# joeyee/Onet

Measured on AMD Instinct MI355X. Metric: training images/sec (twin 256x256 pass), higher is better.
Workload: dtype f32

## Files before the change

### onet_amd/_lib.py

```python
from __future__ import annotations

import ctypes
import os
import re

HERE = os.path.dirname(os.path.abspath(__file__))
HEADER = os.path.join(os.path.dirname(HERE), "include", "onet_hip.h")
EVAL_HEADER = os.path.join(os.path.dirname(HERE), "include", "onet_hip_eval.h")
RAGGED_HEADER = os.path.join(os.path.dirname(HERE), "include", "onet_hip_ragged.h")
RAGGED_SPLIT_HEADER = os.path.join(os.path.dirname(HERE), "include", "onet_hip_ragged_split.h")
ANYMAP_HEADER = os.path.join(os.path.dirname(HERE), "include", "onet_hip_anymap.h")
PAIRS_HEADER = os.path.join(os.path.dirname(HERE), "include", "onet_hip_pairs.h")
UPMAP_HEADER = os.path.join(os.path.dirname(HERE), "include", "onet_hip_upmap.h")
SPLIT_PAIRS_HEADER = os.path.join(os.path.dirname(HERE), "include", "onet_hip_split_pairs.h")
OPTIM_HEADER = os.path.join(os.path.dirname(HERE), "include", "onet_hip_optim.h")
LIBPATH = os.environ.get("ONET_HIP_LIB") or os.path.join(HERE, "libonet_hip.so")

_CT = {
    "int": ctypes.c_int,
    "int64_t": ctypes.c_int64,
    "uint64_t": ctypes.c_uint64,
    "float": ctypes.c_float,
    "double": ctypes.c_double,
}


def parse_header(path: str = HEADER):
    src = open(path).read()
    src = re.sub(r"/\*.*?\*/", " ", src, flags=re.S)
    src = re.sub(r"//[^\n]*", " ", src)
    src = re.sub(r"^\s*#.*$", " ", src, flags=re.M)
    protos = {}
    for m in re.finditer(r"((?:const\s+)?\w+\s*\*?)\s*(onet_\w+)\s*\(([^)]*)\)\s*;", src):
        ret, name, args = m.group(1).strip(), m.group(2), m.group(3).strip()
        if ret.endswith("*"):
            restype = ctypes.c_char_p if "char" in ret else ctypes.c_void_p
        else:
            restype = _CT[ret]
        argtypes, argnames = [], []
        if args and args != "void":
            for a in args.split(","):
                a = a.strip()
                mm = re.match(r"(?:const\s+)?(\w+)\s*(\*?)\s*(\w+)$", a)
                if not mm:
                    raise ValueError(f"cannot parse argument {a!r} of {name}")
                base, ptr, an = mm.groups()
                argtypes.append(ctypes.c_void_p if ptr else _CT[base])
                argnames.append(an)
        protos[name] = (restype, argtypes, argnames)
    return protos


class OnetHipError(RuntimeError):
    pass


_lib = None
_protos = None


def load(build_if_missing: bool = True):
    global _lib, _protos
    if _lib is not None:
        return _lib
    if not os.path.exists(LIBPATH):
        if not build_if_missing:
            raise OnetHipError(f"{LIBPATH} not built; run `python -m onet_amd.build`")
        from . import build as _build
        _build.build()
    lib = ctypes.CDLL(LIBPATH)
    _protos = {}
    for header in (HEADER, EVAL_HEADER, RAGGED_HEADER, RAGGED_SPLIT_HEADER, ANYMAP_HEADER, PAIRS_HEADER, UPMAP_HEADER, SPLIT_PAIRS_HEADER, OPTIM_HEADER):
        protos = parse_header(header)
        for name, (restype, argtypes, _) in protos.items():
            try:
                fn = getattr(lib, name)
            except AttributeError as e:
                raise OnetHipError(f"libonet_hip.so does not export {name} declared in {os.path.basename(header)}") from e
            fn.restype = restype
            fn.argtypes = argtypes
        _protos.update(protos)
    _lib = lib
    return lib


def last_error() -> str:
    return load().onet_last_error().decode()


PROFILE_HOOK = None


def call(name: str, *args, nbytes=None):
    lib = load()
    hook = PROFILE_HOOK
    tok = hook.begin() if hook is not None else None
    rc = getattr(lib, name)(*args)
    if tok is not None:
        hook.end(name, nbytes, tok)
    if rc != 0:
        raise OnetHipError(f"{name} failed ({rc}): {lib.onet_last_error().decode()}")
    return rc
```

### onet_amd/build.py

```python
import os
import subprocess
import sys

HERE = os.path.dirname(os.path.abspath(__file__))
CSRC = os.path.join(HERE, "csrc")
LIB = os.path.join(HERE, "libonet_hip.so")
SOURCES = ["abi.cpp", "conv_mfma.hip", "conv_wino4.hip", "conv_wino4w.hip", "conv_split.hip", "convt_gemm.hip", "stem.hip", "bn.hip", "spatial.hip", "head_loss.hip", "optim.hip", "evalside.hip", "clutter.hip"]
ARCH = "gfx950"


def _stale():
    if not os.path.exists(LIB):
        return True
    t = os.path.getmtime(LIB)
    deps = [os.path.join(CSRC, f) for f in os.listdir(CSRC) if f.endswith((".hip", ".cpp", ".hpp"))] + \
        [os.path.join(HERE, "..", "include", h) for h in ("onet_hip.h", "onet_hip_eval.h", "onet_hip_ragged.h", "onet_hip_ragged_split.h", "onet_hip_anymap.h", "onet_hip_pairs.h", "onet_hip_upmap.h", "onet_hip_split_pairs.h", "onet_hip_optim.h")]
    return any(os.path.getmtime(d) > t for d in deps)


def build(force=False, verbose=False, variant=None, flags=()):
    lib = LIB if variant is None else os.path.join(HERE, f"libonet_hip_{variant}.so")
    if variant is None and not force and not _stale():
        return LIB
    hipcc = os.environ.get("HIPCC", "/opt/rocm/bin/hipcc")
    objdir = CSRC if variant is None else os.path.join(CSRC, "_" + variant)
    os.makedirs(objdir, exist_ok=True)
    objs = []
    procs = []
    for src in SOURCES:
        obj = os.path.join(objdir, src.rsplit(".", 1)[0] + ".o")
        cmd = [hipcc, "-x", "hip", f"--offload-arch={ARCH}", "-O3", "-fPIC", "-std=c++17", "-Wall",
               "-Wno-unused-result", "-fno-slp-vectorize", *flags, "-c", os.path.join(CSRC, src), "-o", obj]
        if verbose:
            cmd.insert(-4, "-Rpass-analysis=kernel-resource-usage")
        procs.append((src, subprocess.Popen(cmd, stdout=subprocess.PIPE, stderr=subprocess.STDOUT, text=True)))
        objs.append(obj)
    failed = False
    for src, p in procs:
        out, _ = p.communicate()
        if p.returncode != 0:
            failed = True
            sys.stderr.write(f"[onet_amd.build] {src} failed:\n{out}\n")
        elif verbose or out.strip():
            sys.stderr.write(out)
    if failed:
        raise RuntimeError("hipcc failed building libonet_hip.so")
    subprocess.check_call([hipcc, "-shared", "-fPIC", f"--offload-arch={ARCH}", "-o", lib] + objs)
    return lib


if __name__ == "__main__":
    if "--variant" in sys.argv:
        i = sys.argv.index("--variant")
        print(build(variant=sys.argv[i + 1], flags=[a for a in sys.argv[i + 2:]]))
    else:
        print(build(force="--force" in sys.argv, verbose="-v" in sys.argv))
```

### onet_amd/csrc/conv_split.hip

```cpp
#include <algorithm>
#include <cstdlib>
#include "common.hpp"
#include "../../include/onet_hip_ragged.h"
#include "../../include/onet_hip_ragged_split.h"
#include "../../include/onet_hip_anymap.h"
#include "../../include/onet_hip_pairs.h"
#include "../../include/onet_hip_split_pairs.h"

using namespace onet;

typedef float f32x16 __attribute__((ext_vector_type(16)));
typedef __bf16 bf16x8 __attribute__((ext_vector_type(8)));
typedef __bf16 bf16x2 __attribute__((ext_vector_type(2)));
typedef unsigned int u32x4s __attribute__((ext_vector_type(4)));
typedef float f32x4s __attribute__((ext_vector_type(4)));

namespace {

constexpr unsigned OOB_S = 0x80000000u;

__device__ __forceinline__ __amdgpu_buffer_rsrc_t s_rsrc(const void* base, int64_t bytes) {
    const int n = bytes > 0x7fffffffll ? 0x7fffffff : (int)bytes;
    return __builtin_amdgcn_make_buffer_rsrc(const_cast<void*>(base), 0, n, 0x00020000);
}
// ... 383 lines not shown
            }
            __syncthreads();
            buf ^= 1;
        }

        if constexpr (F16) {
#pragma unroll
            for (int m = 0; m < 2; ++m)
#pragma unroll
                for (int n = 0; n < NT; ++n)
#pragma unroll
                    for (int r = 0; r < 16; ++r) acc[m][n][r] *= acc_scale;
        }
        const auto [co0, tx, ty, b, y0, x0] = sp_tile(tile, a.coTiles, a.tilesX, a.tilesY);
        if constexpr (ST) {
            float* sc = reinterpret_cast<float*>(lds + 2 * BUF);
            constexpr float npw = (float)(NT * 32), inv_npw = 1.f / npw;
#pragma unroll
            for (int m = 0; m < 2; ++m)
#pragma unroll
                for (int r = 0; r < 16; ++r) {
                    const int piv = __builtin_bit_cast(int, acc[m][0][r]);
                    const float p0 = __builtin_bit_cast(float, __builtin_amdgcn_readlane(piv, 0));
                    const float p1 = __builtin_bit_cast(float, __builtin_amdgcn_readlane(piv, 32));
                    const float pv = kh ? p1 : p0;
                    float s1 = 0.f, s2 = 0.f;
#pragma unroll
                    for (int n = 0; n < NT; ++n) {
                        const float d = acc[m][n][r] - pv;
                        s1 += d;
                        s2 = fmaf(d, d, s2);
                    }
                    s1 = sp_half_sum(s1);
                    s2 = sp_half_sum(s2);
                    if (l31 == 31) {
                        const int cl = m * 32 + (r & 3) + 8 * (r >> 2) + 4 * kh;
                        sc[(wn * 64 + cl) * 2] = fmaf(s1, inv_npw, pv);
                        sc[(wn * 64 + cl) * 2 + 1] = fmaxf(fmaf(-s1 * inv_npw, s1, s2), 0.f);
                    }
                }
            __syncthreads();
            if (tid < 64 && co0 + tid < a.Cout) {
                float mw[8], qw[8];
#pragma unroll
                for (int w = 0; w < 8; ++w) {
                    mw[w] = sc[(w * 64 + tid) * 2];
                    qw[w] = sc[(w * 64 + tid) * 2 + 1];
                }
                const float mean = 0.125f * (((mw[0] + mw[1]) + (mw[2] + mw[3])) + ((mw[4] + mw[5]) + (mw[6] + mw[7])));
                float m2 = ((qw[0] + qw[1]) + (qw[2] + qw[3])) + ((qw[4] + qw[5]) + (qw[6] + qw[7]));
#pragma unroll
                for (int w = 0; w < 8; ++w) m2 = fmaf(npw * (mw[w] - mean), mw[w] - mean, m2);
                const int64_t nblk = (int64_t)a.B * a.tilesY * a.tilesX;
                const int64_t blk = ((int64_t)b * a.tilesY + ty) * a.tilesX + tx;
                float* sp = a.stats + ((int64_t)(co0 + tid) * nblk + blk) * 3;
                sp[0] = 8.f * npw;
                sp[1] = mean;
                sp[2] = m2;
            }
            __syncthreads();
        }
        float* zb = a.z + (int64_t)b * a.z_bs;
        const int xo = x0 + l31;
#pragma unroll
        for (int m = 0; m < 2; ++m)
#pragma unroll
            for (int n = 0; n < NT; ++n) {
                const int yo = y0 + wn * NT + n;
                if (yo < a.H && xo < a.W) {
#pragma unroll
                    for (int r = 0; r < 16; ++r) {
                        const int co = co0 + m * 32 + (r & 3) + 8 * (r >> 2) + 4 * kh;
                        if (co < a.Cout) zb[(int64_t)co * HW + (int64_t)yo * a.W + xo] = acc[m][n][r];
                    }
                }
            }
    }
}


typedef int i32x4s __attribute__((ext_vector_type(4)));
__device__ __forceinline__ i32x4s sp_rsrc4(const void* base, int64_t bytes) {
    const uint64_t p = reinterpret_cast<uint64_t>(base);
    i32x4s r;
    r.x = (int)(p & 0xffffffffu);
    r.y = (int)((p >> 32) & 0xffffu);
    r.z = bytes > 0x7fffffffll ? 0x7fffffff : (int)bytes;
    r.w = 0x00020000;
    return r;
}
__device__ __forceinline__ void sp_dma16(i32x4s rsrc, unsigned lds_base, unsigned voff, unsigned soff) {
    unsigned keep;
    asm volatile("s_nop 4\n\ts_mov_b32 %0, m0\n\ts_mov_b32 m0, %3\n\ts_nop 0\n\tbuffer_load_dwordx4 %1, %2, %4 offen lds\n\ts_mov_b32 m0, %0"
                 : "=&s"(keep)
                 : "v"(voff), "s"(rsrc), "s"(lds_base), "s"(soff)
                 : "memory");
}

__global__ void split_pack_act_kernel(const float* __restrict__ x, int64_t x_bs, unsigned* __restrict__ xs, int64_t xs_bs, int B, int C8,
                                      int H, int W, int f16, float scale, const unsigned* __restrict__ slots) {
    if (slots) {
        float inv;
        scale *= amax_scale(amax_read(slots), false, inv);
    }
    const int64_t n = (int64_t)B * C8 * H * W;
    for (int64_t i = blockIdx.x * (int64_t)blockDim.x + threadIdx.x; i < n; i += (int64_t)gridDim.x * blockDim.x) {
        const int xx = (int)(i % W);
        int64_t r = i / W;
        const int y = (int)(r % H);
        r /= H;
        const int c8 = (int)(r % C8), b = (int)(r / C8);
        const float* src = x + (int64_t)b * x_bs + ((int64_t)c8 * 8 * H + y) * W + xx;
        u32x4s hi, mid;
#pragma unroll
        for (int c = 0; c < 4; ++c) {
            const float va = src[(int64_t)(2 * c) * H * W] * scale, vb = src[(int64_t)(2 * c + 1) * H * W] * scale;
            unsigned h, m;
            if (f16 == 1) split2h(va, vb, h, m);
            else split2(va, vb, h, m);
            hi[c] = h;
            mid[c] = m;
        }
        if (f16 == 2) {
            reinterpret_cast<u32x4s*>(xs + (int64_t)b * xs_bs)[((int64_t)c8 * H + y) * W + xx] = hi;
            continue;
        }
        u32x4s* dst = reinterpret_cast<u32x4s*>(xs + (int64_t)b * xs_bs) + (((int64_t)c8 * H + y) * 2) * W + xx;
        dst[0] = hi;
        dst[W] = mid;
    }
}

struct SpPreArgs {
    const void* xs;
    int64_t xs_bs;
    const __bf16* wq;
    float* z;
    int64_t z_bs;
    int B, Cin, Cout, H, W, tilesX, tilesY, coTiles;
    float* stats;
    const unsigned* x_slots;
    int x_always;
    const unsigned* x_slots2;
    int split_ch;
    const float* rd_z = nullptr;
    union { int64_t rd_z_bs = 0; int64_t pl_y_bs; };
    const float* rd_save = nullptr;
    union { int rd_gimg = 0; int n_img; };
    float* rd_rec = nullptr;
    unsigned* rd_amax = nullptr;
    int z16 = 0, rd_z16 = 0;
    void* zP = nullptr;
    int64_t zP_bs = 0;
    int zP_ch0 = 0;
    const unsigned* zP_slots = nullptr;
    const float* act_save = nullptr;
    unsigned* act_amax = nullptr;
    float* act_a = nullptr;
    int64_t act_a_bs = 0;
    union { const float* hd_L = nullptr; void* pl_P; };
    union { int64_t hd_L_bs = 0; int64_t pl_P_bs; };
    union { float* hd_V = nullptr; float* pl_y; };
};

template <bool W16> struct SpPreCfg {
    static constexpr int NW = 8, NT = 16 / NW, TW = 32, CO_T = 64, ROWS = NW * NT;
    static constexpr int IN_ROWS = ROWS + 2, IN_COLS = W16 ? 36 : 34;
    static constexpr int NPIX = IN_ROWS * IN_COLS;
    static constexpr int NPIXP = W16 ? 656 : 640;
    static constexpr int W_PART = 9 * 2 * CO_T, W_SLOTS = 2 * W_PART, NWI = (W_SLOTS + NW * 64 - 1) / (NW * 64);
    static constexpr int IN_PART = 2 * NPIXP;
    static constexpr int BUF_SLOTS = W_SLOTS + 2 * IN_PART;
    static constexpr int LDS_BYTES = 2 * BUF_SLOTS * 16;
    static constexpr int NB = (NT - 1) + 3;
    static constexpr int LAST_TAP = 4;
    static_assert(CO_T == SpCfg::CO_T && ROWS == SpCfg::ROWS && TW == SpCfg::TW, "sp_tile: one tile shape for every kernel of the family");
};
template <int CTRL> __device__ __forceinline__ float dpp_max(float x) {
    return fmaxf(x, __builtin_bit_cast(float, __builtin_amdgcn_update_dpp(0, __builtin_bit_cast(int, x), CTRL, 0xf, 0xf, false)));
}
template <bool ST, int PM, bool W16, bool ACT = false, bool POOL = false, bool RAG = false>
__global__ __launch_bounds__(SpPreCfg<W16>::NW * 64, SpPreCfg<W16>::NW / 4) void conv3x3_split_pre_kernel(SpPreArgs a) {
    constexpr bool F16 = PM == 1;
    static_assert(!RAG || ACT, "conv3x3_split_pre_kernel: the ragged instance is the activation epilogue's (masked exact maximum)");
    static_assert(!ACT || (PM == 1 && !ST && (!W16 || (RAG && !POOL))),
                  "conv3x3_split_pre_kernel: the activation epilogue goes with the fp16 slot store; on image-pair tiles: the masked record, no pooled twin");
    static_assert(!POOL || ACT, "conv3x3_split_pre_kernel: the pooled stores ride on the activation epilogue");
    using C = SpPreCfg<W16>;
    constexpr bool PAIRS = W16 && ACT;
    constexpr int NT = C::NT, IN_COLS = C::IN_COLS, NWI = C::NWI, CO_T = C::CO_T, NPIXP = C::NPIXP, NB = C::NB;
    constexpr int BUF = C::BUF_SLOTS, W_PART = C::W_PART, IN_PART = C::IN_PART;
    constexpr int NWV = C::NW, NTH = NWV * 64;
    constexpr int NII = (2 * IN_PART + NTH - 1) / NTH;
    extern __shared__ __attribute__((aligned(16))) unsigned char smem_s[];
    u32x4s* lds = reinterpret_cast<u32x4s*>(smem_s);

    int t_first, t_end, t_stride;
    sp_tile_range(a.tilesX * a.tilesY * a.B * a.coTiles, t_first, t_end, t_stride);
    if (t_first >= t_end) return;

    const int tid = threadIdx.x, lane = tid & 63, wn = __builtin_amdgcn_readfirstlane(tid >> 6);
    const int l31 = lane & 31, kh = lane >> 5;
    const int HW = a.H * a.W;
    const int nchunks = PM == 2 ? a.Cin >> 5 : a.Cin >> 4;

    const i32x4s wr = sp_rsrc4(a.wq, (int64_t)a.Cin * (PM == 2 ? 1 : 2) * 9 * a.Cout * 2);
    float xs_inv = 1.f, xs_inv2 = 1.f;
    (void)amax_scale(amax_read(a.x_slots), a.x_always != 0, xs_inv);
    (void)amax_scale(amax_read(a.x_slots2), a.x_always != 0, xs_inv2);
    const int split_chunk = a.split_ch ? (PM == 2 ? a.split_ch >> 5 : a.split_ch >> 4) : 0;
    const float grp_ratio = split_chunk ? xs_inv / xs_inv2 : 1.f;
    const float acc_scale = (split_chunk ? xs_inv2 : xs_inv) * (F16 ? reinterpret_cast<const float*>(a.wq + (int64_t)a.Cin * 2 * 9 * a.Cout)[1] : 1.f);
    const unsigned in_step = (unsigned)(16 * HW * 4), w_step = (unsigned)(2 * 9 * 2 * a.Cout * 16);
    const unsigned lds0 = (unsigned)(uintptr_t)(__attribute__((address_space(3))) unsigned char*)smem_s;

    unsigned in_off[NII], w_off[NWI];
    i32x4s xr;
    int st_tile = t_first, st_chunk = 0;
    unsigned cin_bytes = 0, cw_bytes = 0;
    auto setup_stage = [&]() __attribute__((always_inline)) {
        const bool live = st_tile < t_end;
        const auto [co0, tx, ty, b, y0, x0] = sp_tile(live ? st_tile : t_first, a.coTiles, a.tilesX, a.tilesY);
        const bool img1 = !PAIRS || 2 * b + 1 < a.n_img;
        xr = sp_rsrc4(reinterpret_cast<const unsigned*>(a.xs) + (int64_t)(W16 ? 2 * b : b) * a.xs_bs,
                      (W16 && img1 ? a.xs_bs * 4 : 0) + (int64_t)a.Cin * HW * (PM == 2 ? 2 : 4));
#pragma unroll
        for (int k = 0; k < NII; ++k) {
            const int i = (wn + NWV * k) * 64 + lane;
            const int ph = i / NPIXP, pix = i % NPIXP;
            const int r = pix / IN_COLS, c = pix % IN_COLS;
            const int img = W16 ? c / 18 : 0;
            const int yy = y0 - 1 + r, xx = W16 ? c % 18 - 1 : x0 - 1 + c;
            const bool ok = live && i < 2 * IN_PART && pix < C::NPIX && yy >= 0 && yy < a.H && xx >= 0 && xx < a.W && (!PAIRS || img == 0 || img1);
            const unsigned io = W16 ? (unsigned)(img * a.xs_bs * 4) : 0u;
            in_off[k] = !ok ? OOB_S : PM == 2 ? io + (unsigned)(((ph * a.H + yy) * a.W + xx) * 16)
                                              : io + (unsigned)(((((ph & 1) * a.H + yy) * 2 + (ph >> 1)) * a.W + xx) * 16);
        }
#pragma unroll
        for (int k = 0; k < NWI; ++k) {
            const int i = tid + NTH * k;
            const int co = i & (CO_T - 1), pth = i >> 6;
            const bool ok = live && (i < C::W_SLOTS) && (co0 + co < a.Cout);
            w_off[k] = ok ? (unsigned)((pth * a.Cout + co0 + co) * 16) : OOB_S;
        }
    };
    auto advance = [&]() __attribute__((always_inline)) {
        ++st_chunk;
        cin_bytes += in_step;
        cw_bytes += w_step;
        if (st_chunk == nchunks) {
            st_chunk = 0;
            cin_bytes = cw_bytes = 0;
            st_tile += t_stride;
            setup_stage();
        }
    };
    auto dma_in = [&](int buf, int k) __attribute__((always_inline)) {
        if ((wn + NWV * k) * 64 < 2 * IN_PART)
            sp_dma16(xr, lds0 + (unsigned)((buf * BUF + C::W_SLOTS + (wn + NWV * k) * 64) * 16), in_off[k], cin_bytes);
    };
    auto dma_w = [&](int buf, int k) __attribute__((always_inline)) {
        if (k < NWI - 1 || wn < (C::W_SLOTS - NTH * (NWI - 1)) / 64)
            sp_dma16(wr, lds0 + (unsigned)((buf * BUF + (wn + NWV * k) * 64) * 16), w_off[k], cw_bytes);
    };

    const u32x4s* const a_ptr = lds + kh * CO_T + l31;
    const u32x4s* const b_ptr = lds + C::W_SLOTS + kh * NPIXP + (wn * NT) * IN_COLS + (W16 ? (l31 >> 4) * 18 + (l31 & 15) : l31);

    setup_stage();
#pragma unroll
    for (int k = 0; k < NII; ++k) dma_in(0, k);
#pragma unroll
    for (int k = 0; k < NWI; ++k) dma_w(0, k);
    asm volatile("s_waitcnt vmcnt(0)" ::: "memory");
    __syncthreads();
    int buf = 0;
    float zP_scale = 1.f;
    if constexpr (PM == 1 && !ST && (!W16 || ACT)) {
        float zinv;
        if (a.zP) zP_scale = amax_scale(amax_read(a.zP_slots), !ACT, zinv);
    }
    [[maybe_unused]] float* const act_cf = reinterpret_cast<float*>(lds + 2 * BUF);
    [[maybe_unused]] float cf_next = 0.f;
    [[maybe_unused]] int cf_par = 0;
    auto act_fetch = [&](int t) __attribute__((always_inline)) {
        if (tid < 192 && t < t_end) {
            const int k = tid >> 6;
            cf_next = a.act_save[(int64_t)(k + (k > 0)) * a.Cout + sp_tile(t, a.coTiles, a.tilesX, a.tilesY).co0 + (tid & 63)];
        }
    };
    if constexpr (ACT) act_fetch(t_first);
    for (int tile = t_first; tile < t_end; tile += t_stride) {
        if constexpr (ACT) {
            cf_par ^= 1;
            if (tid < 192) act_cf[cf_par * 192 + tid] = cf_next;
            act_fetch(tile + t_stride);
        }
        f32x16 acc[2][NT];
#pragma unroll
        for (int m = 0; m < 2; ++m)
#pragma unroll
            for (int n = 0; n < NT; ++n)
#pragma unroll
                for (int r = 0; r < 16; ++r) acc[m][n][r] = 0.f;

        for (int c = 0; c < nchunks; ++c) {
            if (split_chunk && c == split_chunk && grp_ratio != 1.f) {
#pragma unroll
                for (int m = 0; m < 2; ++m)
#pragma unroll
                    for (int n = 0; n < NT; ++n)
#pragma unroll
// ... 155 lines not shown
                            const float v = fmaxf(fmaf(acc[m][n][4 * g + j] - mean[j], sc[j], sh[j]), 0.f);
                            acc[m][n][4 * g + j] = v;
                            if constexpr (RAG) vrow[n] = fmaxf(vrow[n], v);
                            else vmax = fmaxf(vmax, v);
                        }
                }
            if constexpr (RAG) {
#pragma unroll
                for (int n = 0; n < NT; ++n)
                    if (img_ok && y0 + wn * NT + n < a.H && xo < a.W) vmax = fmaxf(vmax, vrow[n]);
            }
            if (a.act_amax) {
#pragma unroll
                for (int o = 32; o > 0; o >>= 1) vmax = fmaxf(vmax, __shfl_xor(vmax, o, 64));
                if (lane == 0 && vmax == vmax)
                    atomicMax(a.act_amax + ((tile * NWV + wn) & (AMAX_SLOTS - 1)) * AMAX_STRIDE, __builtin_bit_cast(unsigned, vmax));
            }
            if (a.act_a) {
                float* ab = a.act_a + (int64_t)img * a.act_a_bs;
#pragma unroll
                for (int m = 0; m < 2; ++m)
#pragma unroll
                    for (int n = 0; n < NT; ++n) {
                        const int yo = y0 + wn * NT + n;
                        if (img_ok && yo < a.H && xo < a.W) {
#pragma unroll
                            for (int r = 0; r < 16; ++r) {
                                const int co = co0 + m * 32 + (r & 3) + 8 * (r >> 2) + 4 * kh;
                                if (co < a.Cout) ab[(int64_t)co * HW + (int64_t)yo * a.W + xo] = acc[m][n][r];
                            }
                        }
                    }
            }
        }
        if constexpr (PM == 1 && !ST && (!W16 || ACT)) {
            if (ACT || (a.zP && co0 >= a.zP_ch0)) {
                const float zs = zP_scale;
                u32x4s* zp = reinterpret_cast<u32x4s*>(reinterpret_cast<unsigned*>(a.zP) + (int64_t)img * a.zP_bs);
#pragma unroll
                for (int m = 0; m < 2; ++m)
#pragma unroll
                    for (int n = 0; n < NT; ++n) {
                        const int yo = y0 + wn * NT + n;
#pragma unroll
                        for (int e = 0; e < 2; ++e) {
                            float v[8];
#pragma unroll
                            for (int j = 0; j < 4; ++j) {
                                const float f0 = acc[m][n][8 * e + j], f1 = acc[m][n][8 * e + 4 + j];
                                const unsigned d0 = __builtin_bit_cast(unsigned, f0);
                                const unsigned d1 = __builtin_bit_cast(unsigned, f1);
                                const auto sw = __builtin_amdgcn_permlane32_swap(d0, d1, false, false);
                                const unsigned lo = sw[0], hi4 = sw[1];
                                v[j] = __builtin_bit_cast(float, lo);
                                v[4 + j] = __builtin_bit_cast(float, hi4);
                            }
                            u32x4s hi, mid;
#pragma unroll
                            for (int k = 0; k < 4; ++k) {
                                unsigned hh, mm;
                                split2h_s(v[2 * k], v[2 * k + 1], zs, hh, mm);
                                hi[k] = hh;
                                mid[k] = mm;
                            }
                            if (img_ok && yo < a.H && xo < a.W) {
                                const int c8 = ((co0 - a.zP_ch0 + m * 32) >> 3) + 2 * e + kh;
                                u32x4s* d = zp + ((int64_t)(c8 * a.H + yo) * 2) * a.W + xo;
                                d[0] = hi;
                                d[a.W] = mid;
                            }
                        }
                    }
                if constexpr (POOL) {
                    const int Hp = a.H >> 1, Wp = a.W >> 1, yp = (y0 >> 1) + wn, xp = (x0 + l31) >> 1;
                    const bool pst = (l31 & 1) == 0 && yp < Hp && xp < Wp;
                    u32x4s* const yP = reinterpret_cast<u32x4s*>(reinterpret_cast<unsigned*>(a.pl_P) + (int64_t)b * a.pl_P_bs);
                    float* const yF = a.pl_y + (int64_t)b * a.pl_y_bs;
#pragma unroll
                    for (int m = 0; m < 2; ++m)
#pragma unroll
                        for (int e = 0; e < 2; ++e) {
                            float v[8];
#pragma unroll
                            for (int j = 0; j < 4; ++j) {
                                const float t0 = acc[m][0][8 * e + j], u0 = acc[m][1][8 * e + j];
                                const float t1 = acc[m][0][8 * e + 4 + j], u1 = acc[m][1][8 * e + 4 + j];
                                const float f0 = dpp_max<0xB1>(fmaxf(t0, u0)), f1 = dpp_max<0xB1>(fmaxf(t1, u1));
                                if (a.pl_y && pst) {
                                    const int co = co0 + m * 32 + 16 * e + 4 * kh + j;
                                    yF[((int64_t)co * Hp + yp) * Wp + xp] = f0;
                                    yF[((int64_t)(co + 8) * Hp + yp) * Wp + xp] = f1;
                                }
                                const unsigned d0 = __builtin_bit_cast(unsigned, f0);
                                const unsigned d1 = __builtin_bit_cast(unsigned, f1);
                                const auto sw = __builtin_amdgcn_permlane32_swap(d0, d1, false, false);
                                const unsigned lo = sw[0], hi4 = sw[1];
                                v[j] = __builtin_bit_cast(float, lo);
                                v[4 + j] = __builtin_bit_cast(float, hi4);
                            }
                            u32x4s hi, mid;
#pragma unroll
                            for (int k = 0; k < 4; ++k) {
                                unsigned hh, mm;
                                split2h_s(v[2 * k], v[2 * k + 1], zs, hh, mm);
                                hi[k] = hh;
                                mid[k] = mm;
                            }
                            if (a.pl_P && pst) {
                                const int c8 = ((co0 + m * 32) >> 3) + 2 * e + kh;
                                u32x4s* d = yP + ((int64_t)(c8 * Hp + yp) * 2) * Wp + xp;
                                d[0] = hi;
                                d[Wp] = mid;
                            }
                        }
                }
                continue;
            }
        }
#pragma unroll
        for (int m = 0; m < 2; ++m)
#pragma unroll
            for (int n = 0; n < NT; ++n) {
                const int yo = y0 + wn * NT + n;
                if (yo < a.H && xo < a.W) {
#pragma unroll
                    for (int r = 0; r < 16; ++r) {
                        const int co = co0 + m * 32 + (r & 3) + 8 * (r >> 2) + 4 * kh;
                        if (co < a.Cout) zb[(int64_t)co * HW + (int64_t)yo * a.W + xo] = acc[m][n][r];
                    }
                }
            }
    }
}


template <int CTRL> __device__ __forceinline__ float dpp_add(float x) {
    return x + __builtin_bit_cast(float, __builtin_amdgcn_update_dpp(0, __builtin_bit_cast(int, x), CTRL, 0xf, 0xf, false));
}
__device__ __forceinline__ u32x4s pre16_slot_transpose(const f32x4s& d1, const f32x4s& d2, int c8) {
    const unsigned a0 = pack2bf(d1[0], d1[1]), a1 = pack2bf(d1[2], d1[3]);
    const unsigned b0 = pack2bf(d2[0], d2[1]), b1 = pack2bf(d2[2], d2[3]);
    const bool o1 = (c8 & 1) != 0, o2 = (c8 & 2) != 0, o4 = (c8 & 4) != 0;
    auto st1 = [&](unsigned x) {
        const unsigned y = (unsigned)__shfl_xor((int)x, 1, 64);
        return o1 ? ((y >> 16) | (x & 0xffff0000u)) : ((x & 0xffffu) | (y << 16));
    };
    const unsigned A0 = st1(a0), A1 = st1(a1), B0 = st1(b0), B1 = st1(b1);
    const unsigned ra = (unsigned)__shfl_xor((int)(o2 ? A0 : A1), 2, 64), rb = (unsigned)__shfl_xor((int)(o2 ? B0 : B1), 2, 64);
    const unsigned ka = o2 ? A1 : A0, kb = o2 ? B1 : B0;
    const unsigned Alo = o2 ? ra : ka, Ahi = o2 ? ka : ra, Blo = o2 ? rb : kb, Bhi = o2 ? kb : rb;
    const unsigned r0 = (unsigned)__shfl_xor((int)(o4 ? Alo : Blo), 4, 64), r1 = (unsigned)__shfl_xor((int)(o4 ? Ahi : Bhi), 4, 64);
    return o4 ? u32x4s{r0, r1, Blo, Bhi} : u32x4s{Alo, Ahi, r0, r1};
}
template <bool ST, int PM, bool W16, bool RD = false, bool ACT = false, bool HEAD = false, bool POOL = false, bool RAG = false, bool ANY = false>
__global__ __launch_bounds__(512, 2) void conv3x3_pre16_kernel(SpPreArgs a) {
    constexpr bool F16 = PM == 1;
    static_assert(!ANY || (ACT && PM == 2 && !RAG), "conv3x3_pre16_kernel: the any-map instance is the one-part activation epilogue's");
    static_assert(!POOL || ACT, "conv3x3_pre16_kernel: the pooled stores ride on the activation epilogue");
    static_assert(!RAG || (POOL && PM == 2), "conv3x3_pre16_kernel: the ragged instance is the one-part pooled epilogue's");
    static_assert(!ACT || (PM == 2 && !ST && !RD && (!W16 || !(POOL || RAG || ANY))),
                  "conv3x3_pre16_kernel: the activation epilogue goes with the one-part bf16 slot store; on image-pair tiles: no pooled, ragged or any-map twin");
    static_assert(!HEAD || (PM != 0 && !ST && !W16 && !RD && !ACT), "conv3x3_pre16_kernel: the head epilogue replaces every store of a plain forward launch");
    using C = SpPreCfg<W16>;
    static_assert(C::NW == 8 && C::NT == 2, "conv3x3_pre16_kernel: 8 waves of 2 rows");
    constexpr int NT = 2, IN_COLS = C::IN_COLS, NWI = C::NWI, CO_T = C::CO_T, NPIXP = C::NPIXP;
    constexpr int BUF = C::BUF_SLOTS, IN_PART = C::IN_PART;
    constexpr int NII = (2 * IN_PART + 511) / 512;
    constexpr int CH_OFF = W16 ? 18 : 16;
    constexpr int NSTEP = PM == 2 ? 9 : 14;
    constexpr bool PAIRS = W16 && ACT;
    extern __shared__ __attribute__((aligned(16))) unsigned char smem_s[];
    u32x4s* lds = reinterpret_cast<u32x4s*>(smem_s);

    int t_first, t_end, t_stride;
    sp_tile_range(a.tilesX * a.tilesY * a.B * a.coTiles, t_first, t_end, t_stride);
    if (t_first >= t_end) return;

    const int tid = threadIdx.x, lane = tid & 63, wn = __builtin_amdgcn_readfirstlane(tid >> 6);
    const int r16 = lane & 15, lq = lane >> 4, hq = lq & 1, gq = lq >> 1;
    const int HW = a.H * a.W;
    const int nchunks = PM == 2 ? a.Cin >> 5 : a.Cin >> 4;

    const i32x4s wr = sp_rsrc4(a.wq, (int64_t)a.Cin * (PM == 2 ? 1 : 2) * 9 * a.Cout * 2);
    float xs_inv = 1.f, xs_inv2 = 1.f;
    (void)amax_scale(amax_read(a.x_slots), a.x_always != 0, xs_inv);
    (void)amax_scale(amax_read(a.x_slots2), a.x_always != 0, xs_inv2);
    const int split_chunk = a.split_ch ? (PM == 2 ? a.split_ch >> 5 : a.split_ch >> 4) : 0;
    const float grp_ratio = split_chunk ? xs_inv / xs_inv2 : 1.f;
    const float acc_scale = (split_chunk ? xs_inv2 : xs_inv) * (F16 ? reinterpret_cast<const float*>(a.wq + (int64_t)a.Cin * 2 * 9 * a.Cout)[1] : 1.f);
    const unsigned in_step = (unsigned)(16 * HW * 4), w_step = (unsigned)(2 * 9 * 2 * a.Cout * 16);
    const unsigned lds0 = (unsigned)(uintptr_t)(__attribute__((address_space(3))) unsigned char*)smem_s;

    unsigned in_off[NII], w_off[NWI];
    i32x4s xr;
    int st_tile = t_first, st_chunk = 0;
    unsigned cin_bytes = 0, cw_bytes = 0;
    auto setup_stage = [&]() __attribute__((always_inline)) {
        const bool live = st_tile < t_end;
        const auto [co0, tx, ty, b, y0, x0] = sp_tile(live ? st_tile : t_first, a.coTiles, a.tilesX, a.tilesY);
        const bool img1 = !PAIRS || 2 * b + 1 < a.n_img;
        xr = sp_rsrc4(reinterpret_cast<const unsigned*>(a.xs) + (int64_t)(W16 ? 2 * b : b) * a.xs_bs,
                      (W16 && img1 ? a.xs_bs * 4 : 0) + (int64_t)a.Cin * HW * (PM == 2 ? 2 : 4));
#pragma unroll
        for (int k = 0; k < NII; ++k) {
            const int i = (wn + 8 * k) * 64 + lane;
            const int ph = i / NPIXP, pix = i % NPIXP;
            const int r = pix / IN_COLS, c = pix % IN_COLS;
            const int img = W16 ? c / 18 : 0;
            const int yy = y0 - 1 + r, xx = W16 ? c % 18 - 1 : x0 - 1 + c;
            const bool ok = live && i < 2 * IN_PART && pix < C::NPIX && yy >= 0 && yy < a.H && xx >= 0 && xx < a.W && (!PAIRS || img == 0 || img1);
            const unsigned io = W16 ? (unsigned)(img * a.xs_bs * 4) : 0u;
            in_off[k] = !ok ? OOB_S : PM == 2 ? io + (unsigned)(((ph * a.H + yy) * a.W + xx) * 16)
                                              : io + (unsigned)(((((ph & 1) * a.H + yy) * 2 + (ph >> 1)) * a.W + xx) * 16);
        }
#pragma unroll
        for (int k = 0; k < NWI; ++k) {
            const int i = tid + 512 * k;
            const int co = i & (CO_T - 1), pth = i >> 6;
            const bool ok = live && (i < C::W_SLOTS) && (co0 + co < a.Cout);
            w_off[k] = ok ? (unsigned)((pth * a.Cout + co0 + co) * 16) : OOB_S;
        }
    };
    auto advance = [&]() __attribute__((always_inline)) {
        ++st_chunk;
        cin_bytes += in_step;
        cw_bytes += w_step;
        if (st_chunk == nchunks) {
            st_chunk = 0;
            cin_bytes = cw_bytes = 0;
            st_tile += t_stride;
            setup_stage();
        }
    };
    auto dma_in = [&](int buf, int k) __attribute__((always_inline)) {
        if ((wn + 8 * k) * 64 < 2 * IN_PART)
            sp_dma16(xr, lds0 + (unsigned)((buf * BUF + C::W_SLOTS + (wn + 8 * k) * 64) * 16), in_off[k], cin_bytes);
    };
    auto dma_w = [&](int buf, int k) __attribute__((always_inline)) {
        if (k < NWI - 1 || wn < (C::W_SLOTS - 512 * (NWI - 1)) / 64)
            sp_dma16(wr, lds0 + (unsigned)((buf * BUF + (wn + 8 * k) * 64) * 16), w_off[k], cw_bytes);
    };

    const int xrow0 = (wn * NT) * IN_COLS + r16;
    const u32x4s* const xa_p = lds + C::W_SLOTS + (PM == 2 ? lq : hq) * NPIXP + xrow0;
    const u32x4s* const xh_p = lds + C::W_SLOTS + (2 + hq) * NPIXP + xrow0 + gq;
    const u32x4s* const xv_p = lds + C::W_SLOTS + (2 + hq) * NPIXP + xrow0 + gq * IN_COLS + 2;
    const u32x4s* const xs_p = lds + C::W_SLOTS + (2 + hq) * NPIXP + xrow0 + 2;
    const u32x4s* const wa_p = lds + (gq * 9 * 2 + hq) * CO_T + r16;
    const u32x4s* const wh_p = lds + (gq * 2 + hq) * CO_T + r16;
    const u32x4s* const wv_p = lds + ((3 * gq + 2) * 2 + hq) * CO_T + r16;
    const u32x4s* const ws_p = gq == 0 ? lds + (8 * 2 + hq) * CO_T + r16 : lds + C::W_SLOTS + C::NPIX;
    const int ws_ct = gq == 0 ? 16 : 0;

    setup_stage();
#pragma unroll
    for (int k = 0; k < NII; ++k) dma_in(0, k);
#pragma unroll
    for (int k = 0; k < NWI; ++k) dma_w(0, k);
    asm volatile("s_waitcnt vmcnt(0)" ::: "memory");
    __syncthreads();
    int buf = 0;
    [[maybe_unused]] float* const act_cf = reinterpret_cast<float*>(lds + 2 * BUF);
    [[maybe_unused]] float cf_next = 0.f;
    [[maybe_unused]] int cf_par = 0;
    auto act_fetch = [&](int t) __attribute__((always_inline)) {
        if (tid < 192 && t < t_end) {
            const int k = tid >> 6;
            cf_next = a.act_save[(int64_t)(k + (k > 0)) * a.Cout + sp_tile(t, a.coTiles, a.tilesX, a.tilesY).co0 + (tid & 63)];
        }
    };
    if constexpr (ACT || HEAD) act_fetch(t_first);
    for (int tile = t_first; tile < t_end; tile += t_stride) {
        if constexpr (ACT || HEAD) {
            cf_par ^= 1;
            if (tid < 192) act_cf[cf_par * 192 + tid] = cf_next;
            act_fetch(tile + t_stride);
        }
        f32x4s acc[4][NT][2];
#pragma unroll
        for (int ct = 0; ct < 4; ++ct)
#pragma unroll
            for (int n = 0; n < NT; ++n)
#pragma unroll
                for (int ch = 0; ch < 2; ++ch) acc[ct][n][ch] = f32x4s{0.f, 0.f, 0.f, 0.f};

        for (int c = 0; c < nchunks; ++c) {
            if (split_chunk && c == split_chunk && grp_ratio != 1.f) {
#pragma unroll
                for (int ct = 0; ct < 4; ++ct)
#pragma unroll
                    for (int n = 0; n < NT; ++n)
#pragma unroll
                        for (int ch = 0; ch < 2; ++ch) acc[ct][n][ch] *= grp_ratio;
            }
            const int bo = buf * BUF;
            u32x4s Xp[2][NT + 2][2], Wf[2][4];
            auto load_x = [&](int ph, int f) __attribute__((always_inline)) {
                const int j = f >> 1, ch = f & 1, p = ph & 1;
                if (ph < 3) Xp[p][j][ch] = xa_p[bo + j * IN_COLS + ch * CH_OFF + ph];
                else if (ph == 3) Xp[p][j][ch] = xh_p[bo + j * IN_COLS + ch * CH_OFF];
                else if (j < NT) Xp[p][j][ch] = xv_p[bo + j * IN_COLS + ch * CH_OFF];
                else Xp[p][j][ch] = xs_p[bo + j * IN_COLS + ch * CH_OFF];
            };
            auto load_w = [&](int s) __attribute__((always_inline)) {
#pragma unroll
                for (int ct = 0; ct < 4; ++ct) {
                    if (s < 9) Wf[s & 1][ct] = wa_p[bo + ((s % 3) * 3 + s / 3) * 2 * CO_T + ct * 16];
                    else if (s < 12) Wf[s & 1][ct] = wh_p[bo + (s - 9) * 6 * CO_T + ct * 16];
                    else if (s == 12) Wf[s & 1][ct] = wv_p[bo + ct * 16];
                    else Wf[s & 1][ct] = ws_p[bo + ct * ws_ct];
                }
            };
#pragma unroll
            for (int f = 0; f < 2 * (NT + 2); ++f) load_x(0, f);
            load_w(0);
#pragma unroll
            for (int s = 0; s < NSTEP; ++s) {
                const int ph = s < 9 ? s / 3 : (s < 12 ? 3 : 4);
                const int ro = s < 9 ? s % 3 : (s < 12 ? s - 9 : (s == 12 ? 0 : NT));
                if (s + 1 < NSTEP) load_w(s + 1);
                if (s < 12 && ph + 1 < (PM == 2 ? 3 : 5)) {
#pragma unroll
                    for (int f = 0; f < 2 * (NT + 2); ++f)
// ... 16 lines not shown
                for (int ct = 0; ct < 4; ++ct)
#pragma unroll
                    for (int n = 0; n < NT; ++n)
#pragma unroll
                        for (int ch = 0; ch < 2; ++ch) {
                            if constexpr (F16)
                                acc[ct][n][ch] = __builtin_amdgcn_mfma_f32_16x16x32_f16(__builtin_bit_cast(f16x8, Xp[ph & 1][ro + n][ch]),
                                                                                        __builtin_bit_cast(f16x8, Wf[s & 1][ct]), acc[ct][n][ch], 0, 0, 0);
                            else
                                acc[ct][n][ch] = __builtin_amdgcn_mfma_f32_16x16x32_bf16(__builtin_bit_cast(bf16x8, Xp[ph & 1][ro + n][ch]),
                                                                                         __builtin_bit_cast(bf16x8, Wf[s & 1][ct]), acc[ct][n][ch], 0, 0, 0);
                        }
                __builtin_amdgcn_sched_barrier(0);
            }
            asm volatile("s_waitcnt vmcnt(0)" ::: "memory");
            __syncthreads();
            buf ^= 1;
        }

#pragma unroll
        for (int ct = 0; ct < 4; ++ct)
#pragma unroll
            for (int n = 0; n < NT; ++n)
#pragma unroll
                for (int ch = 0; ch < 2; ++ch) acc[ct][n][ch] *= acc_scale;
        const auto [co0, tx, ty, b, y0, x0] = sp_tile(tile, a.coTiles, a.tilesX, a.tilesY);
        if constexpr (ST) {
            float* sc = reinterpret_cast<float*>(lds + (buf ^ 1) * BUF);
            constexpr float npw = (float)(NT * 32);
#pragma unroll
            for (int ct = 0; ct < 4; ++ct) {
                const float pv = acc[ct][0][0][0];
                float s1 = 0.f, s2 = 0.f;
#pragma unroll
                for (int n = 0; n < NT; ++n)
#pragma unroll
                    for (int ch = 0; ch < 2; ++ch)
#pragma unroll
                        for (int r = 0; r < 4; ++r) {
                            const float d = acc[ct][n][ch][r] - pv;
                            s1 += d;
                            s2 = fmaf(d, d, s2);
                        }
                float mean = fmaf(s1, 1.f / 16.f, pv), m2 = fmaxf(fmaf(-s1 * (1.f / 16.f), s1, s2), 0.f), cnt = 16.f;
#pragma unroll
                for (int o = 16; o <= 32; o <<= 1) {
                    const float mo = __shfl_xor(mean, o, 64), qo = __shfl_xor(m2, o, 64);
                    const float dlt = mo - mean;
                    m2 = (m2 + qo) + (0.5f * cnt) * dlt * dlt;
                    mean = 0.5f * (mean + mo);
                    cnt *= 2.f;
                }
                if (lq == 0) {
                    sc[(wn * 64 + ct * 16 + r16) * 2] = mean;
                    sc[(wn * 64 + ct * 16 + r16) * 2 + 1] = m2;
                }
            }
            __syncthreads();
            if (tid < 64 && co0 + tid < a.Cout) {
                float mw[8], qw[8];
#pragma unroll
                for (int w = 0; w < 8; ++w) {
                    mw[w] = sc[(w * 64 + tid) * 2];
                    qw[w] = sc[(w * 64 + tid) * 2 + 1];
                }
                const float mean = 0.125f * (((mw[0] + mw[1]) + (mw[2] + mw[3])) + ((mw[4] + mw[5]) + (mw[6] + mw[7])));
                float m2 = ((qw[0] + qw[1]) + (qw[2] + qw[3])) + ((qw[4] + qw[5]) + (qw[6] + qw[7]));
#pragma unroll
                for (int w = 0; w < 8; ++w) m2 = fmaf(npw * (mw[w] - mean), mw[w] - mean, m2);
                const int64_t nblk = (int64_t)a.B * a.tilesY * a.tilesX;
                const int64_t blk = ((int64_t)b * a.tilesY + ty) * a.tilesX + tx;
                float* sp = a.stats + ((int64_t)(co0 + tid) * nblk + blk) * 3;
                sp[0] = 8.f * npw;
                sp[1] = mean;
                sp[2] = m2;
            }
            __syncthreads();
        }
        if constexpr (ACT) {
            const float* cf = act_cf + cf_par * 192;
            float vmax = 0.f;
#pragma unroll
            for (int ct = 0; ct < 4; ++ct) {
                const float mean = cf[ct * 16 + r16], sc = cf[64 + ct * 16 + r16], sh = cf[128 + ct * 16 + r16];
#pragma unroll
                for (int n = 0; n < NT; ++n)
#pragma unroll
                    for (int ch = 0; ch < 2; ++ch)
#pragma unroll
                        for (int r = 0; r < 4; ++r) {
                            const float v = fmaxf(fmaf(acc[ct][n][ch][r] - mean, sc, sh), 0.f);
                            acc[ct][n][ch][r] = v;
                            vmax = fmaxf(vmax, v);
                        }
            }
            if (a.act_amax) {
#pragma unroll
                for (int o = 32; o > 0; o >>= 1) vmax = fmaxf(vmax, __shfl_xor(vmax, o, 64));
                if (lane == 0 && vmax == vmax)
                    atomicMax(a.act_amax + ((tile * 8 + wn) & (AMAX_SLOTS - 1)) * AMAX_STRIDE, __builtin_bit_cast(unsigned, vmax));
            }
        }
        if constexpr (HEAD) {
            f32x4s lr[4][NT][2];
            const float* Lb = a.hd_L + (int64_t)b * a.hd_L_bs;
#pragma unroll
            for (int ct = 0; ct < 4; ++ct)
#pragma unroll
                for (int n = 0; n < NT; ++n)
#pragma unroll
                    for (int ch = 0; ch < 2; ++ch) {
                        const int co = co0 + ct * 16 + r16, yo = y0 + wn * NT + n, xo = x0 + 16 * ch + 4 * lq;
                        f32x4s ll = {0.f, 0.f, 0.f, 0.f};
                        if (co < a.Cout && yo < a.H && xo < a.W) ll = *reinterpret_cast<const f32x4s*>(Lb + (int64_t)co * HW + (int64_t)yo * a.W + xo);
                        lr[ct][n][ch] = ll;
                    }
            __builtin_amdgcn_sched_barrier(0);
            const float* cf = act_cf + cf_par * 192;
            f32x4s v[NT][2];
#pragma unroll
            for (int n = 0; n < NT; ++n)
#pragma unroll
                for (int ch = 0; ch < 2; ++ch) v[n][ch] = f32x4s{0.f, 0.f, 0.f, 0.f};
#pragma unroll
            for (int ct = 0; ct < 4; ++ct) {
                const float mean = cf[ct * 16 + r16], sc = cf[64 + ct * 16 + r16], sh = cf[128 + ct * 16 + r16];
#pragma unroll
                for (int n = 0; n < NT; ++n)
#pragma unroll
                    for (int ch = 0; ch < 2; ++ch)
#pragma unroll
                        for (int r = 0; r < 4; ++r)
                            v[n][ch][r] = fmaf(lr[ct][n][ch][r], fmaxf(fmaf(acc[ct][n][ch][r] - mean, sc, sh), 0.f), v[n][ch][r]);
            }
#pragma unroll
            for (int n = 0; n < NT; ++n)
#pragma unroll
                for (int ch = 0; ch < 2; ++ch)
#pragma unroll
                    for (int r = 0; r < 4; ++r)
                        v[n][ch][r] = dpp_add<0x140>(dpp_add<0x141>(dpp_add<0x4E>(dpp_add<0xB1>(v[n][ch][r]))));
            float* Vb = a.hd_V + (int64_t)b * HW;
#pragma unroll
            for (int n = 0; n < NT; ++n)
#pragma unroll
                for (int ch = 0; ch < 2; ++ch) {
                    const int yo = y0 + wn * NT + n, xo = x0 + 16 * ch + 4 * lq;
                    if (r16 == 2 * n + ch && yo < a.H && xo < a.W) *reinterpret_cast<f32x4s*>(Vb + (int64_t)yo * a.W + xo) = v[n][ch];
                }
            continue;
        }
        f32x4s zr[4][NT][2];
        const float* rd_sv = nullptr;
        if constexpr (RD) {
            const int img0 = W16 ? 2 * b : b;
            rd_sv = a.rd_save + (int64_t)(a.rd_gimg ? img0 / a.rd_gimg : 0) * 4 * a.Cout;
#pragma unroll
            for (int ct = 0; ct < 4; ++ct)
#pragma unroll
                for (int n = 0; n < NT; ++n)
#pragma unroll
                    for (int ch = 0; ch < 2; ++ch) {
                        const int co = co0 + ct * 16 + r16, yo = y0 + wn * NT + n, xo = (W16 ? 0 : x0 + 16 * ch) + 4 * lq;
                        f32x4s zz = {0.f, 0.f, 0.f, 0.f};
                        if (co < a.Cout && yo < a.H && xo < a.W) {
                            const int64_t zo = (int64_t)(W16 ? img0 + ch : img0) * a.rd_z_bs + (int64_t)co * HW + (int64_t)yo * a.W + xo;
                            if (a.rd_z16) {
                                const uint2 u = *reinterpret_cast<const uint2*>(reinterpret_cast<const __bf16*>(a.rd_z) + zo);
                                zz = f32x4s{__builtin_bit_cast(float, u.x << 16), __builtin_bit_cast(float, u.x & 0xffff0000u),
                                            __builtin_bit_cast(float, u.y << 16), __builtin_bit_cast(float, u.y & 0xffff0000u)};
                            } else {
                                zz = *reinterpret_cast<const f32x4s*>(a.rd_z + zo);
                            }
                        }
                        zr[ct][n][ch] = zz;
                    }
            __builtin_amdgcn_sched_barrier(0);
        }
        {
            const int half = r16 >> 3, c8 = r16 & 7;
            float* zb = a.z + (int64_t)(W16 ? 2 * b + half : b) * a.z_bs;
            const int xo = (W16 ? 0 : x0 + 16 * half) + 4 * lq;
#pragma unroll
            for (int n = 0; n < NT; ++n) {
                const int yo = y0 + wn * NT + n;
#pragma unroll
                for (int ct = 0; ct < 4; ++ct) {
                    const i32x4s va = __builtin_bit_cast(i32x4s, acc[ct][n][0]), vb = __builtin_bit_cast(i32x4s, acc[ct][n][1]);
                    const i32x4s e1 = {__builtin_amdgcn_update_dpp(va.x, vb.x, 0x128, 0xf, 0xc, false), __builtin_amdgcn_update_dpp(va.y, vb.y, 0x128, 0xf, 0xc, false),
                                       __builtin_amdgcn_update_dpp(va.z, vb.z, 0x128, 0xf, 0xc, false), __builtin_amdgcn_update_dpp(va.w, vb.w, 0x128, 0xf, 0xc, false)};
                    const i32x4s e2 = {__builtin_amdgcn_update_dpp(vb.x, va.x, 0x128, 0xf, 0x3, false), __builtin_amdgcn_update_dpp(vb.y, va.y, 0x128, 0xf, 0x3, false),
                                       __builtin_amdgcn_update_dpp(vb.z, va.z, 0x128, 0xf, 0x3, false), __builtin_amdgcn_update_dpp(vb.w, va.w, 0x128, 0xf, 0x3, false)};
                    const f32x4s d1 = __builtin_bit_cast(f32x4s, e1), d2 = __builtin_bit_cast(f32x4s, e2);
                    if constexpr (PM == 2 && !ST && (!W16 || ACT) && !RD) {
                        const int img = PAIRS ? 2 * b + half : b;
                        const bool img_ok = !PAIRS || img < a.n_img;
                        if constexpr (ACT) {
                            if constexpr (ANY || PAIRS) {
                                if (a.act_a && img_ok && yo < a.H && xo < a.W) {
                                    const int co = co0 + ct * 16 + c8;
                                    float* o = a.act_a + (int64_t)img * a.act_a_bs + (int64_t)co * HW + (int64_t)yo * a.W + xo;
#pragma unroll
                                    for (int i = 0; i < 4; ++i)
                                        if (xo + i < a.W) {
                                            if (co < a.Cout) o[i] = d1[i];
                                            if (co + 8 < a.Cout) o[(int64_t)8 * HW + i] = d2[i];
                                        }
                                }
                            } else if (a.act_a && yo < a.H && xo < a.W) {
                                const int co = co0 + ct * 16 + c8;
                                float* o = a.act_a + (int64_t)b * a.act_a_bs + (int64_t)co * HW + (int64_t)yo * a.W + xo;
                                if (co < a.Cout) *reinterpret_cast<f32x4s*>(o) = d1;
                                if (co + 8 < a.Cout) *reinterpret_cast<f32x4s*>(o + (int64_t)8 * HW) = d2;
                            }
                        }
                        if (ACT || (a.zP && co0 >= a.zP_ch0)) {
                            const bool o4 = (c8 & 4) != 0;
                            const u32x4s slot = pre16_slot_transpose(d1, d2, c8);
                            const int xs = (PAIRS ? 0 : x0 + 16 * half) + 4 * lq + (c8 & 3);
                            if (img_ok && yo < a.H && xs < a.W) {
                                const int g8 = ((co0 - a.zP_ch0) >> 3) + 2 * ct + (o4 ? 1 : 0);
                                u32x4s* zp = reinterpret_cast<u32x4s*>(reinterpret_cast<unsigned*>(a.zP) + (int64_t)img * a.zP_bs);
                                zp[((int64_t)g8 * a.H + yo) * a.W + xs] = slot;
                            }
                            continue;
                        }
                    }
                    if (yo < a.H && xo < a.W) {
                        const int co = co0 + ct * 16 + c8;
                        const int64_t off = (int64_t)co * HW + (int64_t)yo * a.W + xo;
                        if (a.z16) {
                            __bf16* o = reinterpret_cast<__bf16*>(a.z) + (int64_t)(W16 ? 2 * b + half : b) * a.z_bs + off;
                            const bf16x2 p0 = {(__bf16)d1[0], (__bf16)d1[1]}, p1 = {(__bf16)d1[2], (__bf16)d1[3]};
                            const bf16x2 q0 = {(__bf16)d2[0], (__bf16)d2[1]}, q1 = {(__bf16)d2[2], (__bf16)d2[3]};
                            if (co < a.Cout) *reinterpret_cast<uint2*>(o) = uint2{__builtin_bit_cast(unsigned, p0), __builtin_bit_cast(unsigned, p1)};
                            if (co + 8 < a.Cout) *reinterpret_cast<uint2*>(o + (int64_t)8 * HW) = uint2{__builtin_bit_cast(unsigned, q0), __builtin_bit_cast(unsigned, q1)};
                        } else {
                            float* o = zb + off;
                            if (co < a.Cout) *reinterpret_cast<f32x4s*>(o) = d1;
                            if (co + 8 < a.Cout) *reinterpret_cast<f32x4s*>(o + (int64_t)8 * HW) = d2;
                        }
                    }
                }
            }
        }
        if constexpr (POOL) {
            const int Hp = a.H >> 1, Wp = a.W >> 1, yp = (y0 >> 1) + wn, xp0 = (x0 >> 1) + 2 * lq;
            f32x4s pm[4];
#pragma unroll
            for (int ct = 0; ct < 4; ++ct)
#pragma unroll
                for (int ch = 0; ch < 2; ++ch) {
                    const f32x4s t = acc[ct][0][ch], u = acc[ct][1][ch];
                    pm[ct][2 * ch] = fmaxf(fmaxf(t[0], t[1]), fmaxf(u[0], u[1]));
                    pm[ct][2 * ch + 1] = fmaxf(fmaxf(t[2], t[3]), fmaxf(u[2], u[3]));
                }
            if constexpr (ANY) {
                if (a.pl_y && yp < Hp) {
#pragma unroll
                    for (int ct = 0; ct < 4; ++ct) {
                        const int co = co0 + ct * 16 + r16;
                        if (co < a.Cout) {
                            float* row = a.pl_y + (int64_t)b * a.pl_y_bs + ((int64_t)co * Hp + yp) * Wp;
#pragma unroll
                            for (int i = 0; i < 4; ++i) {
                                const int xp = xp0 + (i & 1) + (i & 2 ? 8 : 0);
                                if (xp < Wp) row[xp] = pm[ct][i];
                            }
                        }
                    }
                }
            } else if constexpr (RAG) {
                if (a.pl_y && yp < Hp) {
#pragma unroll
                    for (int ct = 0; ct < 4; ++ct) {
                        const int co = co0 + ct * 16 + r16;
                        if (co < a.Cout) {
                            float* row = a.pl_y + (int64_t)b * a.pl_y_bs + ((int64_t)co * Hp + yp) * Wp;
                            if (xp0 + 1 < Wp) *reinterpret_cast<float2*>(row + xp0) = make_float2(pm[ct][0], pm[ct][1]);
                            if (xp0 + 9 < Wp) *reinterpret_cast<float2*>(row + xp0 + 8) = make_float2(pm[ct][2], pm[ct][3]);
                        }
                    }
                }
            } else if (a.pl_y && yp < Hp && xp0 + 9 < Wp) {
#pragma unroll
                for (int ct = 0; ct < 4; ++ct) {
                    const int co = co0 + ct * 16 + r16;
                    float* o = a.pl_y + (int64_t)b * a.pl_y_bs + ((int64_t)co * Hp + yp) * Wp + xp0;
                    if (co < a.Cout) {
                        *reinterpret_cast<float2*>(o) = make_float2(pm[ct][0], pm[ct][1]);
                        *reinterpret_cast<float2*>(o + 8) = make_float2(pm[ct][2], pm[ct][3]);
                    }
                }
            }
            if (a.pl_P) {
                const int c8 = r16 & 7, xs = xp0 + (c8 & 2 ? 8 : 0) + (c8 & 1);
                u32x4s* yP = reinterpret_cast<u32x4s*>(reinterpret_cast<unsigned*>(a.pl_P) + (int64_t)b * a.pl_P_bs);
#pragma unroll
                for (int p = 0; p < 2; ++p) {
                    const u32x4s slot = pre16_slot_transpose(pm[2 * p], pm[2 * p + 1], c8);
                    const int g8 = (co0 >> 3) + 2 * (2 * p + (c8 >> 2)) + (r16 >> 3);
                    if (yp < Hp && xs < Wp) yP[((int64_t)g8 * Hp + yp) * Wp + xs] = slot;
                }
            }
        }
        if constexpr (RD) {
            __builtin_amdgcn_sched_barrier(0);
            float* sc = reinterpret_cast<float*>(lds + (buf ^ 1) * BUF);
            float vmax = 0.f;
#pragma unroll
            for (int ct = 0; ct < 4; ++ct) {
                const int co = co0 + ct * 16 + r16, cc = min(co, a.Cout - 1);
                const float mean = rd_sv[cc], invstd = rd_sv[a.Cout + cc], scl = rd_sv[2 * a.Cout + cc], sh = rd_sv[3 * a.Cout + cc];
                float s1 = 0.f, s2 = 0.f;
#pragma unroll
                for (int n = 0; n < NT; ++n)
#pragma unroll
                    for (int ch = 0; ch < 2; ++ch) {
                        const int yo = y0 + wn * NT + n, xo = (W16 ? 0 : x0 + 16 * ch) + 4 * lq;
                        if (co < a.Cout && yo < a.H && xo < a.W) {
#pragma unroll
                            for (int r = 0; r < 4; ++r) {
                                const float da = acc[ct][n][ch][r], d = zr[ct][n][ch][r] - mean;
                                const float dy = fmaf(d, scl, sh) > 0.f ? da : 0.f;
                                s1 += dy;
                                s2 = fmaf(dy, d * invstd, s2);
                                vmax = fmaxf(vmax, fabsf(da));
                            }
                        }
                    }
                s1 += __shfl_xor(s1, 16, 64);
                s2 += __shfl_xor(s2, 16, 64);
                s1 += __shfl_xor(s1, 32, 64);
                s2 += __shfl_xor(s2, 32, 64);
                if (lq == 0) {
                    sc[(wn * 64 + ct * 16 + r16) * 2] = s1;
                    sc[(wn * 64 + ct * 16 + r16) * 2 + 1] = s2;
                }
            }
            if (a.rd_amax) {
#pragma unroll
                for (int o = 32; o > 0; o >>= 1) vmax = fmaxf(vmax, __shfl_xor(vmax, o, 64));
                if (lane == 0 && vmax == vmax) atomicMax(a.rd_amax + ((blockIdx.x * 8 + wn) & (AMAX_SLOTS - 1)) * AMAX_STRIDE, __builtin_bit_cast(unsigned, vmax));
            }
            __syncthreads();
            if (tid < 64 && co0 + tid < a.Cout) {
                double t1 = 0.0, t2 = 0.0;
#pragma unroll
                for (int w = 0; w < 8; ++w) {
                    t1 += (double)sc[(w * 64 + tid) * 2];
                    t2 += (double)sc[(w * 64 + tid) * 2 + 1];
                }
                const int64_t blk = ((int64_t)b * a.tilesY + ty) * a.tilesX + tx;
                float* o = a.rd_rec + (blk * a.Cout + co0 + tid) * 4;
                o[0] = (float)t1;
                o[1] = (float)(t1 - (double)o[0]);
                o[2] = (float)t2;
                o[3] = (float)(t2 - (double)o[2]);
            }
            __syncthreads();
        }
    }
}

template <class Args>
int sp_launch_persistent(void (*kern)(Args), PerDeviceOnce& once, int lds_bytes, int64_t tiles, int block, const char* name, const Args& a, hipStream_t st) {
    if (once.first()) {
        (void)hipFuncSetAttribute(reinterpret_cast<const void*>(kern), hipFuncAttributeMaxDynamicSharedMemorySize, lds_bytes);
    }
    const int64_t resident = (int64_t)device_cu_count();
    const int64_t blocks = std::min<int64_t>((tiles + 7) / 8 * 8, std::max<int64_t>(8, resident / 8 * 8));
    hipLaunchKernelGGL(kern, dim3((unsigned)blocks), dim3(block), lds_bytes, st, a);
    return check_launch(name);
}

template <bool ST, int PM, bool W16, bool RD = false, bool ACT = false, bool HEAD = false, bool POOL = false, bool RAG = false, bool ANY = false>
int launch_split_pre(SpPreArgs a, hipStream_t st) {
    using C = SpPreCfg<W16>;
    const int LDS_BYTES = C::LDS_BYTES + (ST ? C::NW * 64 * 2 * 4 : 0) + (ACT || HEAD ? 2 * 3 * 64 * 4 : 0);
    a.tilesX = W16 ? 1 : cdiv(a.W, C::TW);
    a.tilesY = cdiv(a.H, C::ROWS);
    a.coTiles = cdiv(a.Cout, C::CO_T);
    if (W16 && ACT) {
        a.n_img = a.B;
        a.B = (a.B + 1) / 2;
    } else if (W16) {
        a.B /= 2;
    }
    const int64_t tiles = (int64_t)a.B * a.tilesX * a.tilesY * a.coTiles;
    ONET_REQUIRE(tiles > 0 && tiles < (1ll << 31), "conv3x3_split_pre: tile count %lld out of range", (long long)tiles);
    constexpr bool P16 = RD || PM == 2 || (ST && !W16) || HEAD;
    void (*kern)(SpPreArgs);
    static_assert(!ANY || P16, "launch_split_pre: the any-map instance exists on the 16x16x32 kernel alone");
    if constexpr (P16) kern = conv3x3_pre16_kernel<ST, PM, W16, RD, ACT, HEAD, POOL, RAG, ANY>;
    else kern = conv3x3_split_pre_kernel<ST, PM, W16, ACT, POOL, RAG>;
    static PerDeviceOnce attr_once;
    return sp_launch_persistent(kern, attr_once, LDS_BYTES, tiles, C::NW * 64,
                                HEAD   ? (PM == 2 ? "conv3x3_pre16_head_kernel" : "conv3x3_split_pre_head_kernel")
                                : POOL ? (PM == 2 ? "conv3x3_pre16_act_pool_kernel" : "conv3x3_split_pre_act_pool_kernel")
                                : ACT  ? (W16 ? (PM == 2 ? "conv3x3_pre16_act_pairs_kernel" : "conv3x3_split_pre_act_pairs_kernel")
                                              : PM == 2 ? "conv3x3_pre16_act_kernel" : "conv3x3_split_pre_act_kernel")
                                      : "conv3x3_split_pre_kernel", a, st);
}

int split_nparts(int B, int H, int W) {
    if (B <= 0 || W < 32 || (W % SpCfg::TW) || (H % SpCfg::ROWS)) return 0;
    const int64_t n = (int64_t)B * (H / SpCfg::ROWS) * (W / SpCfg::TW);
    return n < (1 << 30) ? (int)n : 0;
}

template <bool ST, bool NORM, bool F16>
int launch_split(SpArgs a, hipStream_t st) {
    using C = SpCfg;
    const int LDS_BYTES = C::LDS_BYTES + (ST ? C::NW * 64 * 2 * 4 : 0) + (NORM ? 2 * 2 * 8 * 4 * 4 : 0);
    a.tilesX = cdiv(a.W, C::TW);
    a.tilesY = cdiv(a.H, C::ROWS);
    a.coTiles = cdiv(a.Cout, C::CO_T);
    const int64_t tiles = (int64_t)a.B * a.tilesX * a.tilesY * a.coTiles;
    ONET_REQUIRE(tiles > 0 && tiles < (1ll << 31), "conv3x3_split: tile count %lld out of range", (long long)tiles);
    static PerDeviceOnce attr_once;
    return sp_launch_persistent(conv3x3_split_kernel<ST, NORM, F16>, attr_once, LDS_BYTES, tiles, 512, "conv3x3_split_kernel", a, st);
}

int split_fwd(const float* x, int64_t x_bs, const void* wq, float* z, int64_t z_bs, int B, int Cin, int Cout, int H, int W,
              void* stream, float* stats, int wq_f16, const float* nsave = nullptr, int n_groups = 0, const unsigned* x_amax = nullptr,
              int x_always = 0) {
    ONET_REQUIRE(x && wq && z, "conv3x3_split_fwd: null pointer");
    ONET_REQUIRE(B > 0 && Cin > 0 && Cout > 0 && H > 0 && W > 16, "conv3x3_split_fwd: bad shape (maps wider than 16 pixels)");
    ONET_REQUIRE((Cin % 16) == 0, "conv3x3_split_fwd: Cin must be a multiple of 16 (use onet_conv_fwd)");
    ONET_REQUIRE((W & 3) == 0 && (x_bs & 3) == 0 && (reinterpret_cast<uintptr_t>(x) & 15) == 0,
                 "conv3x3_split_fwd: W %% 4 == 0 and 16-byte aligned image rows required (use onet_conv3x3_winograd4_fwd)");
    ONET_REQUIRE(x_bs >= (int64_t)Cin * H * W && z_bs >= (int64_t)Cout * H * W, "conv3x3_split_fwd: batch stride too small");
    ONET_REQUIRE((int64_t)(Cin + 32) * H * W * 4 < (1ll << 31) && (int64_t)(Cin + 32) * 2 * 9 * Cout * 2 < (1ll << 31),
                 "conv3x3_split_fwd: operand exceeds the 2 GiB buffer-resource range");
    SpArgs a{x, x_bs, (const __bf16*)wq, z, z_bs, B, Cin, Cout, H, W, 0, 0, 0, stats, nsave, 1, x_amax, x_always};
    ONET_REQUIRE(!x_amax || wq_f16, "conv3x3_split: magnitude slots go with the fp16 pack");
    if (stats) ONET_REQUIRE(split_nparts(B, H, W) > 0, "conv3x3_split_fwd_stats: the map must be made of full 16 x 32 tiles");
    if (nsave) {
        ONET_REQUIRE(n_groups > 0 && B % n_groups == 0, "conv3x3_split_fwd_norm: the batch must hold n_groups equal statistics groups");
        a.nimg = B / n_groups;
        if (wq_f16) return stats ? launch_split<true, true, true>(a, as_stream(stream)) : launch_split<false, true, true>(a, as_stream(stream));
        return stats ? launch_split<true, true, false>(a, as_stream(stream)) : launch_split<false, true, false>(a, as_stream(stream));
    }
    if (wq_f16) return stats ? launch_split<true, false, true>(a, as_stream(stream)) : launch_split<false, false, true>(a, as_stream(stream));
    return stats ? launch_split<true, false, false>(a, as_stream(stream)) : launch_split<false, false, false>(a, as_stream(stream));
}


struct SwArgs {
    const float* x;
    int64_t x_bs;
    const float* dz;
    int64_t dz_bs;
    float* slab;
    int B, Cin, Cout, H, W, ciTiles, coTiles, splitK, tilesX;
    const float* nsave;
    int nimg;
    const unsigned* x_amax;
    const unsigned* dz_amax;
};

constexpr int SR_SDZ = 36;
template <int G> struct SwCfg {
    static constexpr int SPG = 8 / G;
    static constexpr int P = G == 1 ? 36 : (G == 2 ? 20 : 12);
    static constexpr int SLOT = G * P;
    static constexpr int SX = 4 * SLOT + 4;
    static constexpr int X_PART = 64 * SX;
    static constexpr int GOFF = G == 1 ? 16 : (G == 2 ? 20 : 24);
    static constexpr int SOFF = G == 4 ? 12 : 8;
};

template <int G, int COT, bool NORM, bool F16>
__global__ __launch_bounds__(512, 2) void conv3x3_split_wgrad_kernel(SwArgs a) {
    using C = SwCfg<G>;
    constexpr int SR_SX = C::SX, SR_SLOT = C::SLOT, SR_X_PART = C::X_PART;
    constexpr int SR_DZ_PART = COT * SR_SDZ;
    constexpr int NSEG = COT == 64 ? 2 : 4;
    constexpr int DZI = COT / 64;
    __shared__ __attribute__((aligned(16))) unsigned dz_lds[2 * 2 * SR_DZ_PART];
    __shared__ __attribute__((aligned(16))) unsigned x_lds[2 * SR_X_PART];

    int bid = xcd_block_id();
    const int tiles = a.ciTiles * a.coTiles;
    const int ks = bid / tiles, tile = bid % tiles;
    const int ci0 = (tile % a.ciTiles) * 64, co0 = (tile / a.ciTiles) * COT;
    const int nunits = (a.B / G) * a.tilesX * a.H;
    const int per = (nunits + a.splitK - 1) / a.splitK;
    const int u0 = ks * per, u1 = min(u0 + per, nunits);

    const int tid = threadIdx.x, lane = tid & 63, wid = tid >> 6;
    const int grp = COT == 64 ? wid >> 2 : 0, wm = COT == 64 ? (wid >> 1) & 1 : wid >> 1, wn = wid & 1;
    const int l31 = lane & 31, kh = lane >> 5;
    const int HW = a.H * a.W;

    f32x16 acc[9];
#pragma unroll
    for (int t = 0; t < 9; ++t)
#pragma unroll
        for (int r = 0; r < 16; ++r) acc[t][r] = 0.f;
    float x_inv = 1.f, dz_inv = 1.f;
    const float x_scale = F16 ? amax_scale(amax_read(a.x_amax), false, x_inv) : 1.f;
    const float dz_scale = F16 ? amax_scale(amax_read(a.dz_amax), true, dz_inv) : 1.f;

    const int st_c = tid >> 3, st_s = tid & 7;
    const int st_sub = st_s / C::SPG, st_w = st_s % C::SPG;
    u32x4s dzv[2 * DZI], xq[2];
    float xh[2];
    float n_mean[2] = {0.f, 0.f}, n_sc[2] = {0.f, 0.f}, n_sh[2] = {0.f, 0.f};
    bool pend_v[4] = {false, false, false, false}, pend_g1 = false;
    if constexpr (NORM) {
        const int ch = min(ci0 + st_c, a.Cin - 1), last = a.B / a.nimg - 1;
#pragma unroll
        for (int g = 0; g < 2; ++g) {
            const float* sv = a.nsave + (int64_t)min(g, last) * 4 * a.Cin + ch;
            n_mean[g] = sv[0];
            n_sc[g] = sv[2 * a.Cin];
            n_sh[g] = sv[3 * a.Cin];
        }
    }
    auto issue_dz = [&](int b, int x0, int y, int p0 = 0, int p1 = 64) __attribute__((always_inline)) {
        const __amdgpu_buffer_rsrc_t dr = G == 1 ? s_rsrc(a.dz + (int64_t)b * a.dz_bs, (int64_t)a.Cout * HW * 4)
                                                 : s_rsrc(a.dz, ((int64_t)(a.B - 1) * a.dz_bs + (int64_t)a.Cout * HW) * 4);
        const int xs = x0 + 8 * st_w;
#pragma unroll
        for (int i = 0; i < DZI; ++i) {
            const int co = co0 + st_c + 64 * i;
            const bool ok = y >= 0 && y < a.H && co < a.Cout;
            const unsigned base = (unsigned)((co * HW + y * a.W + xs) * 4) + (G == 1 ? 0u : (unsigned)((int64_t)(b * G + st_sub) * a.dz_bs * 4));
#pragma unroll
            for (int k = 0; k < 2; ++k)
                if (2 * i + k >= p0 && 2 * i + k < p1)
                    dzv[2 * i + k] = __builtin_amdgcn_raw_buffer_load_b128(dr, (ok && xs + 4 * k < a.W) ? base + 16 * k : OOB_S, 0, 0);
        }
    };
    auto issue_x = [&](int b, int x0, int y, int p0 = 0, int p1 = 64) __attribute__((always_inline)) {
        const __amdgpu_buffer_rsrc_t xr = G == 1 ? s_rsrc(a.x + (int64_t)b * a.x_bs, (int64_t)a.Cin * HW * 4)
                                                 : s_rsrc(a.x, ((int64_t)(a.B - 1) * a.x_bs + (int64_t)a.Cin * HW) * 4);
        const int xs = x0 + 8 * st_w;
        const bool ok = y >= 0 && y < a.H && ci0 + st_c < a.Cin;
        const unsigned base = (unsigned)(((ci0 + st_c) * HW + y * a.W + xs) * 4) + (G == 1 ? 0u : (unsigned)((int64_t)(b * G + st_sub) * a.x_bs * 4));
        if (NORM && p0 == 0) {
            pend_v[0] = ok && xs > 0 && xs - 1 < a.W;
            pend_v[1] = ok && xs < a.W;
            pend_v[2] = ok && xs + 4 < a.W;
            pend_v[3] = ok && st_w == C::SPG - 1 && xs + 8 < a.W;
            pend_g1 = (G == 1 ? b : b * G + st_sub) >= a.nimg;
// ... 507 lines not shown
    if (COT == 128) {
        if (G == 1) ONET_SWP_F(1, 128);
        else if (G == 2) ONET_SWP_F(2, 128);
        else ONET_SWP_F(4, 128);
    } else if (G == 1) ONET_SWP_F(1, 64);
    else if (G == 2) ONET_SWP_F(2, 64);
    else ONET_SWP_F(4, 64);
#undef ONET_SWP_F
#undef ONET_SWP_LAUNCH
    int rc = check_launch("conv3x3_split_wgrad_pre_kernel");
    if (rc) return rc;
    return launch_wgrad_reduce((const float*)ws, dw, a.splitK * slabs, 9, Cout, Cin, 0, accumulate, as_stream(stream));
}

int onet_conv3x3_split_pack_weights(const float* w, void* wq_fwd, void* wq_dgrad, void* amax_ws, int Cout, int Cin, int fwd_f16,
                                    int dgrad_f16, void* stream) {
    ONET_REQUIRE(w && (wq_fwd || wq_dgrad), "conv3x3_split_pack_weights: null pointer");
    ONET_REQUIRE(amax_ws || !(fwd_f16 == 1 || dgrad_f16 == 1), "conv3x3_split_pack_weights: the fp16 packs need the 8 KB magnitude workspace");
    if (fwd_f16 == 1 || dgrad_f16 == 1) {
        (void)hipMemsetAsync(amax_ws, 0, AMAX_SLOTS * AMAX_STRIDE * sizeof(unsigned), as_stream(stream));
        const int64_t nw = (int64_t)Cout * Cin * 9;
        hipLaunchKernelGGL(absmax_slots_kernel, dim3((unsigned)std::min<int64_t>((nw + 1023) / 1024, 1024)), dim3(256), 0, as_stream(stream), w,
                           nw, (unsigned*)amax_ws);
        int rc0 = check_launch("absmax_slots_kernel");
        if (rc0) return rc0;
    }
    ONET_REQUIRE(Cout > 0 && Cin > 0, "conv3x3_split_pack_weights: bad shape");
    ONET_REQUIRE(!wq_fwd || (Cin % 16) == 0, "conv3x3_split_pack_weights: the forward pack needs Cin %% 16 == 0");
    const int64_t n = (int64_t)std::max(Cin, ((Cout + 15) / 16) * 16) * 9 * std::max(Cin, Cout);
    const int blocks = (int)std::min<int64_t>((n + 255) / 256, 8192);
    if (wq_fwd) {
        hipLaunchKernelGGL(pack3x3_split_kernel, dim3(blocks), dim3(256), 0, as_stream(stream), w, (__bf16*)wq_fwd, Cout, Cin, 0, fwd_f16,
                           (const unsigned*)amax_ws);
        int rc = check_launch("pack3x3_split_kernel");
        if (rc) return rc;
    }
    if (wq_dgrad) hipLaunchKernelGGL(pack3x3_split_kernel, dim3(blocks), dim3(256), 0, as_stream(stream), w, (__bf16*)wq_dgrad, Cout, Cin, 1,
                                     dgrad_f16, (const unsigned*)amax_ws);
    return check_launch("pack3x3_split_kernel");
}

int onet_conv3x3_split_fwd(const float* x, int64_t x_bs, const void* wq, int wq_f16, float* z, int64_t z_bs, int B, int Cin, int Cout,
                           int H, int W, void* stream) {
    return split_fwd(x, x_bs, wq, z, z_bs, B, Cin, Cout, H, W, stream, nullptr, wq_f16);
}

int onet_absmax_slots(const float* x, int64_t n, void* slots, void* stream) {
    ONET_REQUIRE(x && slots && n > 0, "absmax_slots: bad args");
    hipLaunchKernelGGL(absmax_slots_kernel, dim3((unsigned)std::min<int64_t>((n + 1023) / 1024, 4096)), dim3(256), 0, as_stream(stream), x, n,
                       (unsigned*)slots);
    return check_launch("absmax_slots_kernel");
}

int onet_conv3x3_split_conv_amax(const float* x, int64_t x_bs, const void* x_amax, int scale_always, const void* wq, float* z, int64_t z_bs,
                                 float* part, int B, int Cin, int Cout, int H, int W, void* stream) {
    return split_fwd(x, x_bs, wq, z, z_bs, B, Cin, Cout, H, W, stream, part, 1, nullptr, 0, (const unsigned*)x_amax, scale_always);
}

int onet_conv3x3_split_wgrad_f16(const float* x, int64_t x_bs, const void* x_amax, const float* save, int n_groups, const float* dz,
                                 int64_t dz_bs, const void* dz_amax, float* dw, void* ws, int64_t ws_bytes, int B, int Cin, int Cout,
                                 int H, int W, int accumulate, void* stream) {
    return split_wgrad_impl(x, x_bs, dz, dz_bs, dw, ws, ws_bytes, B, Cin, Cout, H, W, accumulate, stream, save, save ? n_groups : 0, 1,
                            (const unsigned*)x_amax, (const unsigned*)dz_amax);
}

int onet_conv3x3_split_fwd_norm(const float* z_prev, int64_t z_bs, const float* save, int n_groups, const void* wq, int wq_f16,
                                const void* x_amax, float* z, int64_t zo_bs, float* part, int B, int Cin, int Cout, int H, int W,
                                void* stream) {
    ONET_REQUIRE(save, "conv3x3_split_fwd_norm: null pointer");
    return split_fwd(z_prev, z_bs, wq, z, zo_bs, B, Cin, Cout, H, W, stream, part, wq_f16, save, n_groups, (const unsigned*)x_amax);
}

int onet_split_pack_act(const float* x, int64_t x_bs, void* xs, int64_t xs_bs, int B, int C, int H, int W, int f16, float scale,
                        const void* slots, void* stream) {
    ONET_REQUIRE(x && xs, "split_pack_act: null pointer");
    ONET_REQUIRE(B > 0 && C > 0 && (C % 8) == 0 && H > 0 && W > 0, "split_pack_act: C must be a multiple of 8");
    ONET_REQUIRE((reinterpret_cast<uintptr_t>(xs) & 15) == 0 && (xs_bs & 3) == 0, "split_pack_act: 16-byte aligned slots required");
    const int64_t n = (int64_t)B * (C / 8) * H * W;
    const int blocks = (int)std::min<int64_t>((n + 255) / 256, 1 << 20);
    hipLaunchKernelGGL(split_pack_act_kernel, dim3(blocks), dim3(256), 0, as_stream(stream), x, x_bs, (unsigned*)xs, xs_bs, B, C / 8, H, W,
                       f16, scale, (const unsigned*)slots);
    return check_launch("split_pack_act_kernel");
}

static int pre_operand_checks(const char* entry, const void* xs, int64_t xs_bs, int wq_f16, int Cin, int Cout, int H, int W) {
    ONET_REQUIRE((Cin % (wq_f16 == 2 ? 32 : 16)) == 0, "%s: Cin must be a multiple of 16 (32 for plain bf16 operands)", entry);
    ONET_REQUIRE((xs_bs & 3) == 0 && (reinterpret_cast<uintptr_t>(xs) & 15) == 0, "%s: 16-byte aligned slots required", entry);
    ONET_REQUIRE(xs_bs >= (int64_t)Cin * H * W / (wq_f16 == 2 ? 2 : 1), "%s: batch stride too small", entry);
    ONET_REQUIRE((int64_t)(Cin + 32) * H * W * 4 < (1ll << 31) && (int64_t)(Cin + 32) * 2 * 9 * Cout * 2 < (1ll << 31),
                 "%s: operand exceeds the 2 GiB buffer-resource range", entry);
    ONET_REQUIRE(W != 16 || xs_bs * 4 + (int64_t)Cin * H * W * 4 < (1ll << 31), "%s: image pair exceeds the buffer-resource range", entry);
    return 0;
}

int onet_conv3x3_split_pre_nparts(int B, int H, int W) {
    if (W == 16) return (B > 0 && (B % 2) == 0 && (H % 16) == 0) ? (B / 2) * (H / 16) : 0;
    return split_nparts(B, H, W);
}

int onet_conv3x3_split_fwd_pre(const void* xs, int64_t xs_bs, const void* x_amax, int scale_always, const void* x_amax2, int split_ch,
                               const void* wq, int wq_f16, void* z, int z_bf16, int64_t z_bs, float* part, int B, int Cin, int Cout, int H, int W,
                               void* stream) {
    ONET_REQUIRE(!z_bf16 || (wq_f16 == 2 && (z_bs & 3) == 0 && (reinterpret_cast<uintptr_t>(z) & 7) == 0),
                 "conv3x3_split_fwd_pre: a bf16 output goes with plain bf16 operands (wq_f16 == 2), 8-byte aligned rows");
    ONET_REQUIRE(split_ch >= 0 && split_ch < Cin && (split_ch % 32) == 0, "conv3x3_split_fwd_pre: split_ch must be a multiple of 32 inside Cin");
    ONET_REQUIRE(xs && wq && z, "conv3x3_split_fwd_pre: null pointer");
    ONET_REQUIRE(B > 0 && Cin > 0 && Cout > 0 && H > 0 && (W > 16 || (W == 16 && (B % 2) == 0 && (H % 16) == 0)),
                 "conv3x3_split_fwd_pre: bad shape (maps wider than 16 pixels, or exactly 16 wide with an even batch and H %% 16 == 0)");
    ONET_REQUIRE(wq_f16 != 2 || (W % 4) == 0, "conv3x3_split_fwd_pre: plain bf16 operands need W %% 4 == 0");
    if (const int rc = pre_operand_checks("conv3x3_split_fwd_pre", xs, xs_bs, wq_f16, Cin, Cout, H, W)) return rc;
    ONET_REQUIRE(z_bs >= (int64_t)Cout * H * W, "conv3x3_split_fwd_pre: batch stride too small");
    SpPreArgs a{xs, xs_bs, (const __bf16*)wq, (float*)z, z_bs, B, Cin, Cout, H, W, 0, 0, 0, part, (const unsigned*)x_amax, scale_always,
                (const unsigned*)x_amax2, split_ch};
    a.z16 = z_bf16 ? 1 : 0;
    if (part) ONET_REQUIRE(onet_conv3x3_split_pre_nparts(B, H, W) > 0, "conv3x3_split_fwd_pre: statistics need a map made of full 16 x 32 tiles");
    hipStream_t st = as_stream(stream);
    if (W == 16) {
        if (wq_f16 == 2) return part ? launch_split_pre<true, 2, true>(a, st) : launch_split_pre<false, 2, true>(a, st);
        if (wq_f16) return part ? launch_split_pre<true, 1, true>(a, st) : launch_split_pre<false, 1, true>(a, st);
        return part ? launch_split_pre<true, 0, true>(a, st) : launch_split_pre<false, 0, true>(a, st);
    }
    if (wq_f16 == 2) return part ? launch_split_pre<true, 2, false>(a, st) : launch_split_pre<false, 2, false>(a, st);
    if (wq_f16) return part ? launch_split_pre<true, 1, false>(a, st) : launch_split_pre<false, 1, false>(a, st);
    return part ? launch_split_pre<true, 0, false>(a, st) : launch_split_pre<false, 0, false>(a, st);
}

int onet_conv3x3_split_dgrad_pre_bnreduce(const void* dzs, int64_t dzs_bs, const void* dz_amax, int scale_always, const void* wq, int wq_f16,
                                          float* da, int64_t da_bs, const void* z_prev, int z_bf16, int64_t z_bs, const float* save, int group_images,
                                          float* rec4, void* da_amax, int B, int Cin, int Cout, int H, int W, void* stream) {
    ONET_REQUIRE(dzs && wq && da && z_prev && save && rec4, "conv3x3_split_dgrad_pre_bnreduce: null pointer");
    if (onet_conv3x3_split_pre_nparts(B, H, W) <= 0 || (W != 16 && (W % 32)) || (Cout % 16)) return 1;
    if (W == 16 && ((group_images % 2) || wq_f16 != 2)) return 1;
    if (Cin / (wq_f16 == 2 ? 32 : 16) < 4) return 1;
    ONET_REQUIRE(B > 0 && Cin > 0 && Cout > 0, "conv3x3_split_dgrad_pre_bnreduce: bad shape");
    ONET_REQUIRE(group_images >= 0 && (group_images == 0 || B % group_images == 0), "conv3x3_split_dgrad_pre_bnreduce: bad statistics groups");
    if (const int rc = pre_operand_checks("conv3x3_split_dgrad_pre_bnreduce", dzs, dzs_bs, wq_f16, Cin, Cout, H, W)) return rc;
    ONET_REQUIRE((z_bs & 3) == 0 && (reinterpret_cast<uintptr_t>(z_prev) & (z_bf16 ? 7 : 15)) == 0 && (da_bs & 3) == 0 && (reinterpret_cast<uintptr_t>(da) & 15) == 0,
                 "conv3x3_split_dgrad_pre_bnreduce: 16-byte aligned rows required");
    ONET_REQUIRE(da_bs >= (int64_t)Cout * H * W && z_bs >= (int64_t)Cout * H * W, "conv3x3_split_dgrad_pre_bnreduce: batch stride too small");
    SpPreArgs a{dzs, dzs_bs, (const __bf16*)wq, da, da_bs, B, Cin, Cout, H, W, 0, 0, 0, nullptr, (const unsigned*)dz_amax, scale_always, nullptr, 0};
    a.rd_z = (const float*)z_prev;
    a.rd_z16 = z_bf16 ? 1 : 0;
    a.rd_z_bs = z_bs;
    a.rd_save = save;
    a.rd_gimg = group_images;
    a.rd_rec = rec4;
    a.rd_amax = (unsigned*)da_amax;
    hipStream_t st = as_stream(stream);
    if (W == 16) return launch_split_pre<false, 2, true, true>(a, st);
    if (wq_f16 == 2) return launch_split_pre<false, 2, false, true>(a, st);
    return wq_f16 ? launch_split_pre<false, 1, false, true>(a, st) : launch_split_pre<false, 0, false, true>(a, st);
}

int onet_conv3x3_split_dgrad_pre_slots(const void* dzs, int64_t dzs_bs, const void* dz_amax, int scale_always, const void* wq, int wq_f16,
                                       float* da, int64_t da_bs, void* daP, int64_t daP_bs, int ch0, const void* daP_amax, int B, int Cin,
                                       int Cout, int H, int W, void* stream) {
    ONET_REQUIRE(dzs && wq && da && daP && (daP_amax || wq_f16 == 2) && (wq_f16 == 1 || wq_f16 == 2), "conv3x3_split_dgrad_pre_slots: bad args");
    ONET_REQUIRE(B > 0 && Cin > 0 && Cout > 0 && H > 0 && W >= 32 && (W % 32) == 0 && (H % 16) == 0,
                 "conv3x3_split_dgrad_pre_slots: maps made of full 16 x 32 tiles");
    ONET_REQUIRE(ch0 > 0 && ch0 < Cout && (ch0 % 64) == 0 && (Cout % 64) == 0, "conv3x3_split_dgrad_pre_slots: ch0 and Cout must be multiples of 64");
    if (const int rc = pre_operand_checks("conv3x3_split_dgrad_pre_slots", dzs, dzs_bs, wq_f16, Cin, Cout, H, W)) return rc;
    ONET_REQUIRE((daP_bs & 3) == 0 && (reinterpret_cast<uintptr_t>(daP) & 15) == 0, "conv3x3_split_dgrad_pre_slots: 16-byte aligned slots required");
    ONET_REQUIRE(da_bs >= (int64_t)ch0 * H * W && daP_bs >= (int64_t)(Cout - ch0) * H * W / (wq_f16 == 2 ? 2 : 1),
                 "conv3x3_split_dgrad_pre_slots: batch stride too small");
    SpPreArgs a{dzs, dzs_bs, (const __bf16*)wq, da, da_bs, B, Cin, Cout, H, W, 0, 0, 0, nullptr, (const unsigned*)dz_amax, scale_always, nullptr, 0};
    a.zP = daP;
    a.zP_bs = daP_bs;
    a.zP_ch0 = ch0;
    a.zP_slots = (const unsigned*)daP_amax;
    if (wq_f16 == 2) return launch_split_pre<false, 2, false>(a, as_stream(stream));
    return launch_split_pre<false, 1, false>(a, as_stream(stream));
}

enum class EvMap { Full, Ragged, AnyMap, Pairs };
enum class EvEpi { Act, Pool, Head, Plain };
struct EvalEntry {
    const char* name;
    int parts;
    EvMap map;
    EvEpi epi;
};
struct EvSlots { const void* x_amax = nullptr; int scale_always = 0; const void* x_amax2 = nullptr; int split_ch = 0; };
struct EvAct { void* aP = nullptr; int64_t aP_bs = 0; const void* aP_slots = nullptr; void* a_amax = nullptr; float* a = nullptr; int64_t a_bs = 0; };
struct EvPool { void* yP = nullptr; int64_t yP_bs = 0; float* y = nullptr; int64_t y_bs = 0; };
struct EvHead { const float* L = nullptr; int64_t L_bs = 0; float* V = nullptr; };
struct EvPlain { float* z = nullptr; int64_t z_bs = 0; };
struct EvalConv {
    const void* xs;
    int64_t xs_bs;
    EvSlots in;
    const void* wq;
    const float* save;
    EvAct act;
    EvPool pool;
    EvHead head;
    EvPlain plain;
    int B, Cin, Cout, H, W;
    void* stream;
};

static bool pre_map_ok(bool ragged, int H, int W) {
    if (ragged) return !((H & 1) || (W & 3) || (int64_t)H * W >= (1 << 24));
    return !(W < 32 || (W % 32) || (H % 16));
}

static bool aligned(const void* p, int64_t bs, int bytes) { return !p || ((bs & 3) == 0 && (reinterpret_cast<uintptr_t>(p) & (bytes - 1)) == 0); }

static int eval_conv(const EvalEntry& e, const EvalConv& g) {
    const char* entry = e.name;
    const bool one = e.parts == 1, pool = e.epi == EvEpi::Pool, act = pool || e.epi == EvEpi::Act;
    const int B = g.B, Cin = g.Cin, Cout = g.Cout, H = g.H, W = g.W;
    if (act) ONET_REQUIRE(g.xs && g.wq && g.save && g.act.aP && (g.act.aP_slots || one), "%s: null pointer", entry);
    else if (e.epi == EvEpi::Head) ONET_REQUIRE(g.xs && g.wq && g.save && g.head.L && g.head.V, "%s: null pointer", entry);
    else ONET_REQUIRE(g.xs && g.wq && g.plain.z, "%s: null pointer", entry);
    ONET_REQUIRE(!pool || g.pool.yP || g.pool.y, "%s: a pooled destination is required (yP, y or both)", entry);
    ONET_REQUIRE(B > 0 && Cin > 0 && Cout > 0 && H > 0 && W > 0, "%s: bad shape", entry);
    const int64_t image = (int64_t)(Cin + 32) * H * W * 4, pack = (int64_t)(Cin + 32) * 2 * 9 * Cout * 2;
    EvMap map = e.map;
    if ((Cin % (one ? 32 : 16)) || (e.epi == EvEpi::Head ? Cout != 64 : (Cout % 64))) return 1;
    if (map == EvMap::AnyMap || map == EvMap::Pairs) {
        if (pack >= (1ll << 31) || (one && (g.act.a_amax || (int64_t)H * W >= (1 << 24) || image >= (1ll << 31)))) return 1;
        if (map == EvMap::Pairs && (W > 16 || g.xs_bs > (1ll << 29) || g.xs_bs * 4 + image >= (1ll << 31))) return 1;
        if (map == EvMap::AnyMap && pre_map_ok(true, H, W)) map = EvMap::Ragged;
    } else if (!pre_map_ok(map == EvMap::Ragged, H, W)) {
        return 1;
    }
    ONET_REQUIRE(!(one && map == EvMap::Ragged) || !g.act.a_amax, "%s: the ragged entry records no exact maximum (a_amax must be NULL)", entry);
    ONET_REQUIRE(g.in.split_ch >= 0 && g.in.split_ch < Cin && (g.in.split_ch % 32) == 0, "%s: split_ch must be a multiple of 32 inside Cin", entry);
    if (const int rc = pre_operand_checks(entry, g.xs, g.xs_bs, one ? 2 : 1, Cin, Cout, H, W)) return rc;
    const int64_t n = (int64_t)Cout * H * W, np = (int64_t)Cout * (H >> 1) * (W >> 1), per = one ? 2 : 1;
    if (act) {
        ONET_REQUIRE(aligned(g.act.aP, g.act.aP_bs, 16) && aligned(g.pool.yP, g.pool.yP_bs, 16), "%s: 16-byte aligned slots required", entry);
        if (map == EvMap::AnyMap || map == EvMap::Pairs)
            ONET_REQUIRE(aligned(g.act.a, 0, 4) && aligned(g.pool.y, 0, 4), "%s: 4-byte aligned floats required", entry);
        else if (one || pool)
            ONET_REQUIRE(aligned(g.act.a, g.act.a_bs, 16) && aligned(g.pool.y, g.pool.y_bs, 16), "%s: 16-byte aligned rows required", entry);
        ONET_REQUIRE(g.act.aP_bs >= n / per && (!g.act.a || g.act.a_bs >= n) && (!g.pool.yP || g.pool.yP_bs >= np / per) && (!g.pool.y || g.pool.y_bs >= np),
                     "%s: batch stride too small", entry);
    } else if (e.epi == EvEpi::Head) {
        ONET_REQUIRE(aligned(g.head.L, g.head.L_bs, 16) && aligned(g.head.V, 0, 16), "%s: 16-byte aligned rows required", entry);
        ONET_REQUIRE(g.head.L_bs >= n, "%s: batch stride too small", entry);
    } else {
        ONET_REQUIRE(aligned(g.plain.z, g.plain.z_bs, 16), "%s: 16-byte aligned rows required", entry);
        ONET_REQUIRE(g.plain.z_bs >= n, "%s: batch stride too small", entry);
    }
    SpPreArgs p{g.xs, g.xs_bs, (const __bf16*)g.wq, g.plain.z, g.plain.z_bs, B, Cin, Cout, H, W, 0, 0, 0, nullptr, (const unsigned*)g.in.x_amax,
                g.in.scale_always, (const unsigned*)g.in.x_amax2, g.in.split_ch};
    p.act_save = g.save;
    if (act) {
        p.zP = g.act.aP;
        p.zP_bs = g.act.aP_bs;
        p.zP_ch0 = 0;
        p.zP_slots = (const unsigned*)g.act.aP_slots;
        p.act_amax = (unsigned*)g.act.a_amax;
        p.act_a = g.act.a;
        p.act_a_bs = g.act.a_bs;
    }
    if (pool) {
        p.pl_P = g.pool.yP;
        p.pl_P_bs = g.pool.yP_bs;
        p.pl_y = g.pool.y;
        p.pl_y_bs = g.pool.y_bs;
    } else if (e.epi == EvEpi::Head) {
        p.hd_L = g.head.L;
        p.hd_L_bs = g.head.L_bs;
        p.hd_V = g.head.V;
    }
    hipStream_t st = as_stream(g.stream);
    const bool pairs = map == EvMap::Pairs, any = map == EvMap::AnyMap, rag = map == EvMap::Ragged && !pre_map_ok(false, H, W);
    if (one) {
        if (e.epi == EvEpi::Plain) return launch_split_pre<false, 2, false>(p, st);
        if (e.epi == EvEpi::Head) return launch_split_pre<false, 2, false, false, false, true>(p, st);
        if (pool && any) return launch_split_pre<false, 2, false, false, true, false, true, false, true>(p, st);
        if (pool && rag) return launch_split_pre<false, 2, false, false, true, false, true, true>(p, st);
        if (pool) return launch_split_pre<false, 2, false, false, true, false, true>(p, st);
        if (pairs) return launch_split_pre<false, 2, true, false, true>(p, st);
        if (any) return launch_split_pre<false, 2, false, false, true, false, false, false, true>(p, st);
        return launch_split_pre<false, 2, false, false, true>(p, st);
    }
    if (e.epi == EvEpi::Plain) return launch_split_pre<false, 1, false>(p, st);
    if (e.epi == EvEpi::Head) return launch_split_pre<false, 1, false, false, false, true>(p, st);
    if (pool && rag) return launch_split_pre<false, 1, false, false, true, false, true, true>(p, st);
    if (pool) return launch_split_pre<false, 1, false, false, true, false, true>(p, st);
    if (pairs) return launch_split_pre<false, 1, true, false, true, false, false, true>(p, st);
    if (rag) return launch_split_pre<false, 1, false, false, true, false, false, true>(p, st);
    return launch_split_pre<false, 1, false, false, true>(p, st);
}

int onet_conv3x3_split_fwd_pre_act(const void* xs, int64_t xs_bs, const void* x_amax, int scale_always, const void* x_amax2, int split_ch,
                                   const void* wq, const float* save, void* aP, int64_t aP_bs, const void* aP_slots, void* a_amax, float* a,
                                   int64_t a_bs, int B, int Cin, int Cout, int H, int W, void* stream) {
    return eval_conv({"conv3x3_split_fwd_pre_act", 2, EvMap::Full, EvEpi::Act}, {xs, xs_bs, {x_amax, scale_always, x_amax2, split_ch}, wq, save,
                     {aP, aP_bs, aP_slots, a_amax, a, a_bs}, {}, {}, {}, B, Cin, Cout, H, W, stream});
}

int onet_conv3x3_split_fwd_pre_act_ragged(const void* xs, int64_t xs_bs, const void* x_amax, int scale_always, const void* x_amax2, int split_ch,
                                          const void* wq, const float* save, void* aP, int64_t aP_bs, const void* aP_slots, void* a_amax, float* a,
                                          int64_t a_bs, int B, int Cin, int Cout, int H, int W, void* stream) {
    return eval_conv({"conv3x3_split_fwd_pre_act_ragged", 2, EvMap::Ragged, EvEpi::Act}, {xs, xs_bs, {x_amax, scale_always, x_amax2, split_ch}, wq, save,
                     {aP, aP_bs, aP_slots, a_amax, a, a_bs}, {}, {}, {}, B, Cin, Cout, H, W, stream});
}

int onet_conv3x3_split_fwd_pre_act_pairs(const void* xs, int64_t xs_bs, const void* x_amax, int scale_always, const void* x_amax2, int split_ch,
                                         const void* wq, const float* save, void* aP, int64_t aP_bs, const void* aP_slots, void* a_amax, float* a,
                                         int64_t a_bs, int B, int Cin, int Cout, int H, int W, void* stream) {
    return eval_conv({"conv3x3_split_fwd_pre_act_pairs", 2, EvMap::Pairs, EvEpi::Act}, {xs, xs_bs, {x_amax, scale_always, x_amax2, split_ch}, wq, save,
// ... 178 lines not shown
```

### onet_amd/csrc/stem.hip

```cpp
#include <algorithm>
#include "common.hpp"

using namespace onet;

namespace {

struct StemArgs {
    const float* x;
    int64_t x_bs;
    const float* w;
    float* z;
    int64_t z_bs;
    float* part;
    int B, Cout, H, W, tilesX, tilesY;
    int twin_B;
    float twin_bias;
};

constexpr int ST_TH = 16, ST_TW = 64, ST_LR = ST_TH + 2, ST_LC = ST_TW + 4;
constexpr int ST_MAXC = 128;

#define ONET_ST_DPP_ADD(v, ctrl, rmask) \
    v += __builtin_bit_cast(float, __builtin_amdgcn_update_dpp(0, __builtin_bit_cast(int, v), ctrl, rmask, 0xf, false))
__device__ __forceinline__ float wave_sum_hi(float v) {
    ONET_ST_DPP_ADD(v, 0x128, 0xf);
    ONET_ST_DPP_ADD(v, 0x124, 0xf);
    ONET_ST_DPP_ADD(v, 0x122, 0xf);
    ONET_ST_DPP_ADD(v, 0x121, 0xf);
    ONET_ST_DPP_ADD(v, 0x142, 0xa);
    ONET_ST_DPP_ADD(v, 0x143, 0xc);
    return v;
}
#undef ONET_ST_DPP_ADD

template <int CIN>
__global__ __launch_bounds__(256) void stem_conv_stats_kernel(StemArgs a) {
    __shared__ float tile[CIN][ST_LR][ST_LC];
    __shared__ float sc[4][ST_MAXC][2];
    int bid = blockIdx.x;
    const int tx = bid % a.tilesX;
    bid /= a.tilesX;
    const int ty = bid % a.tilesY;
    const int b = bid / a.tilesY;
    const int y0 = ty * ST_TH, x0 = tx * ST_TW;
    const int tid = threadIdx.x, lane = tid & 63, wid = tid >> 6;
    const int HW = a.H * a.W;
    const bool comp = a.twin_B > 0 && b >= a.twin_B;
    const float* xb = a.x + (int64_t)(comp ? b - a.twin_B : b) * a.x_bs;

    for (int i = tid; i < CIN * ST_LR * 66; i += 256) {
        const int ci = i / (ST_LR * 66), r = (i / 66) % ST_LR, c = i % 66;
        const int yy = y0 - 1 + r, xx = x0 - 1 + c;
        const bool ok = yy >= 0 && yy < a.H && xx >= 0 && xx < a.W;
        float v = ok ? xb[(int64_t)ci * HW + (int64_t)yy * a.W + xx] : 0.f;
        if (comp && ok) v = fminf(fmaxf(1.f - v + a.twin_bias, 0.f), 1.f);
        tile[ci][r][c] = v;
    }
    __syncthreads();

    const int r = tid >> 4, q = tid & 15;
    float win[CIN][3][6];
#pragma unroll
    for (int ci = 0; ci < CIN; ++ci)
#pragma unroll
        for (int dy = 0; dy < 3; ++dy)
#pragma unroll
            for (int dx = 0; dx < 6; ++dx) win[ci][dy][dx] = tile[ci][r + dy][4 * q + dx];

    float* zb = a.z + (int64_t)b * a.z_bs + (int64_t)(y0 + r) * a.W + x0 + 4 * q;
    for (int co = 0; co < a.Cout; ++co) {
        const float* wp = a.w + (int64_t)co * CIN * 9;
        float acc[4] = {0.f, 0.f, 0.f, 0.f};
#pragma unroll
        for (int ci = 0; ci < CIN; ++ci)
#pragma unroll
            for (int dy = 0; dy < 3; ++dy)
#pragma unroll
                for (int dx = 0; dx < 3; ++dx) {
                    const float wv = wp[(ci * 3 + dy) * 3 + dx];
#pragma unroll
                    for (int j = 0; j < 4; ++j) acc[j] = fmaf(wv, win[ci][dy][dx + j], acc[j]);
                }
        *reinterpret_cast<float4*>(zb + (int64_t)co * HW) = make_float4(acc[0], acc[1], acc[2], acc[3]);
        if (a.part) {
            const float pv = __builtin_bit_cast(float, __builtin_amdgcn_readfirstlane(__builtin_bit_cast(int, acc[0])));
            float s1 = 0.f, s2 = 0.f;
#pragma unroll
            for (int j = 0; j < 4; ++j) {
                const float d = acc[j] - pv;
                s1 += d;
                s2 = fmaf(d, d, s2);
            }
            s1 = wave_sum_hi(s1);
            s2 = wave_sum_hi(s2);
            if (lane == 63) {
                sc[wid][co][0] = fmaf(s1, 1.f / 256.f, pv);
                sc[wid][co][1] = fmaxf(fmaf(-s1 * (1.f / 256.f), s1, s2), 0.f);
            }
        }
    }
    if (a.part) {
        __syncthreads();
        if (tid < a.Cout) {
            float mw[4], qw[4];
#pragma unroll
            for (int w = 0; w < 4; ++w) {
                mw[w] = sc[w][tid][0];
                qw[w] = sc[w][tid][1];
            }
            const float mean = 0.25f * ((mw[0] + mw[1]) + (mw[2] + mw[3]));
            float m2 = (qw[0] + qw[1]) + (qw[2] + qw[3]);
#pragma unroll
            for (int w = 0; w < 4; ++w) m2 = fmaf(256.f * (mw[w] - mean), mw[w] - mean, m2);
            const int64_t nblk = (int64_t)a.B * a.tilesY * a.tilesX;
            const int64_t blk = ((int64_t)b * a.tilesY + ty) * a.tilesX + tx;
            float* sp = a.part + ((int64_t)tid * nblk + blk) * 3;
            sp[0] = 1024.f;
            sp[1] = mean;
            sp[2] = m2;
        }
    }
}

int stem_nparts(int B, int Cin, int Cout, int H, int W) {
    if (B <= 0 || Cin < 1 || Cin > 4 || Cout < 1 || Cout > ST_MAXC || H <= 0 || W <= 0 || (H % ST_TH) || (W % ST_TW)) return 0;
    const int64_t n = (int64_t)B * (H / ST_TH) * (W / ST_TW);
    return n < (1 << 30) ? (int)n : 0;
}

}

extern "C" {

int onet_conv3x3_stem_nparts(int B, int Cin, int Cout, int H, int W) { return stem_nparts(B, Cin, Cout, H, W); }

int onet_conv3x3_stem_fwd_stats(const float* x, int64_t x_bs, const float* w, float* z, int64_t z_bs, float* part, int B, int Cin,
                                int Cout, int H, int W, int twin_B, float twin_bias, void* stream) {
    ONET_REQUIRE(x && w && z, "conv3x3_stem_fwd_stats: null pointer");
    ONET_REQUIRE(stem_nparts(B, Cin, Cout, H, W) > 0,
                 "conv3x3_stem_fwd_stats: needs 1 <= Cin <= 4, Cout <= %d and a map made of full 16 x 64 tiles (onet_conv3x3_stem_nparts() == 0 elsewhere)",
                 ST_MAXC);
    ONET_REQUIRE(x_bs >= (int64_t)Cin * H * W && z_bs >= (int64_t)Cout * H * W, "conv3x3_stem_fwd_stats: batch stride too small");
    ONET_REQUIRE((z_bs & 3) == 0 && (reinterpret_cast<uintptr_t>(z) & 15) == 0, "conv3x3_stem_fwd_stats: 16-byte aligned output rows required");
    ONET_REQUIRE(twin_B == 0 || 2 * twin_B == B, "conv3x3_stem_fwd_stats: a twin batch holds twin_B = B / 2 images in memory");
    StemArgs a{x, x_bs, w, z, z_bs, part, B, Cout, H, W, W / ST_TW, H / ST_TH, twin_B, twin_bias};
    const int64_t blocks = (int64_t)B * a.tilesX * a.tilesY;
    const dim3 g((unsigned)blocks), t(256);
    switch (Cin) {
        case 1: hipLaunchKernelGGL(stem_conv_stats_kernel<1>, g, t, 0, as_stream(stream), a); break;
        case 2: hipLaunchKernelGGL(stem_conv_stats_kernel<2>, g, t, 0, as_stream(stream), a); break;
        case 3: hipLaunchKernelGGL(stem_conv_stats_kernel<3>, g, t, 0, as_stream(stream), a); break;
        default: hipLaunchKernelGGL(stem_conv_stats_kernel<4>, g, t, 0, as_stream(stream), a); break;
    }
    return check_launch("stem_conv_stats_kernel");
}

}
```

### onet_amd/functional.py

```python
from __future__ import annotations

import torch

from . import ops


def _carries_settings(cls):
    fwd, bwd = cls.forward, cls.backward

    def forward(ctx, *args, **kw):
        ctx._onet_settings = ops.active_settings()
        return fwd(ctx, *args, **kw)

    def backward(ctx, *grads):
        if torch.is_grad_enabled():
            raise RuntimeError("onet_amd: double differentiation (create_graph=True) is not supported: the HIP backward kernels "
                               "build no graph of their own")
        with ops.using(getattr(ctx, "_onet_settings", None)):
            return bwd(ctx, *grads)

    forward.__doc__, backward.__doc__ = fwd.__doc__, bwd.__doc__
    cls.forward, cls.backward = staticmethod(forward), staticmethod(backward)
    return cls

# ... 15 lines not shown
class ConvBNReLUFn(torch.autograd.Function):

    @staticmethod
    def forward(ctx, x, weight, gamma, beta, running_mean, running_var, training, momentum, eps, packed, out, groups=1,
                link_out=None, link_in=None, aux=None, p16=None):
        ops.require_gpu(x, weight, gamma, beta)
        if p16 is not None and (p16.get("x") is not None or p16.get("want")):
            return ConvBNReLUFn._forward_pre(ctx, x, weight, gamma, beta, running_mean, running_var, training, momentum, eps, packed,
                                             groups, link_out, link_in, p16, aux)
        ctx.pre = False
        want_pool = link_out.pop("want_pool", None) if link_out is not None else None
        defer = bool(link_out.pop("defer", False)) if link_out is not None else False
        defer = defer and training and out is None and want_pool is None
        norm = None
        if link_in is not None and link_in.get("deferred"):
            norm = (link_in["z"], link_in["save"], link_in.get("slots"))
        x_amax = aux.get("x_amax") if (aux is not None and norm is None) else None
        if norm is not None:
            z, cm = ops.conv3x3_fwd_bn_partials(None, packed, norm=norm)
        else:
            z, cm = ops.conv3x3_fwd_bn_partials(x, packed, amax=x_amax) if training else (ops.conv3x3_auto(x, packed, 0, amax=x_amax), None)
        dst = None if out is None else out[0]
        G = groups if (training and groups > 1) else 1
        C = z.shape[1]
        save_all = torch.empty((G, 4, C), dtype=torch.float32, device=z.device)
        Bz, _, Hz, Wz = z.shape
        pooled = None
        a_amax = ops.new_amax(z.device) if (not defer and z.is_cuda and ops.split_f16() and ops.split_enabled()
                                            and ops.conv_algo() in ("auto", "split", "bf16")) else None
        act_slots = ops.new_amax(z.device) if (defer and ops.split_f16()) else None
        if want_pool is not None and ops.FUSE_POOL and Hz % 2 == 0 and Wz % 4 == 0:
            pooled = (torch.empty((Bz, C, Hz // 2, Wz // 2), dtype=torch.float32, device=z.device), None)

        def apply(zg, sv, o, sl):
            nonlocal pooled
            if defer:
                return None
            if pooled is not None:
                if o is None:
                    o = torch.empty_like(zg)
                if ops.bn_relu_apply_pool(zg, sv, o, pooled[0][sl], amax=a_amax):
                    return o
                pooled = None
            return ops.bn_relu_apply(zg, sv, out=o, amax=a_amax)

        if G == 1:
            if training:
                ops.bn_train_coeffs(z, gamma, beta, running_mean, running_var, momentum, eps,
                                    cm=None if cm is None else (cm, 0, cm.shape[1]), save=save_all[0], act_slots=act_slots)
            else:
                ops.bn_eval_coeffs(gamma, beta, running_mean, running_var, eps, save=save_all[0])
            a = apply(z, save_all[0], dst, slice(0, Bz))
            if defer:
                a = ops.fp32_placeholder(z.shape, z.device)
        else:
            B = z.shape[0]
            Bg = B // G
            a = dst if dst is not None else (ops.fp32_placeholder(z.shape, z.device) if defer else torch.empty_like(z))
            for g in range(G):
                zg = z[g * Bg:(g + 1) * Bg]
                npg = 0 if cm is None else cm.shape[1] // G
                ops.bn_train_coeffs(zg, gamma, beta, running_mean, running_var, momentum, eps,
                                    cm=None if cm is None else (cm, g * npg, npg), save=save_all[g], act_slots=act_slots)
                apply(zg, save_all[g], None if defer else a[g * Bg:(g + 1) * Bg], slice(g * Bg, (g + 1) * Bg))
        if aux is not None:
            aux["a_amax"] = a_amax
        ctx.twin = ops.twin_src_of(x)
        below = (link_in.pop("z"), link_in.pop("save")) if (training and link_in is not None and "z" in link_in) else (None, None)
        ctx.save_for_backward(x, z, save_all, None if norm is None else norm[0], None if norm is None else norm[1], *below)
        ctx.training = training
        ctx.packed = packed
        ctx.wshape = tuple(weight.shape)
        _record_versions(ctx, weight, gamma, beta)
        ctx.link_out = ctx.link_in = None
        if training and link_out is not None:
            link_out.clear()
            link_out.update(z=z, save=save_all)
            if defer:
                link_out["deferred"] = True
                link_out["slots"] = act_slots
            ctx.link_out = link_out
        if below[0] is not None:
            ctx.link_in = link_in
        if pooled is not None and link_out is not None:
            link_out["pooled"] = pooled
        return a

    @staticmethod
    def _forward_pre(ctx, x, weight, gamma, beta, running_mean, running_var, training, momentum, eps, packed, groups, link_out,
                     link_in, p16, aux=None):
        want_pool = link_out.pop("want_pool", None) if link_out is not None else None
        if link_out is not None:
            link_out.pop("defer", None)
        xP = p16.get("x")
        x_slots = p16.get("x_slots") if xP is not None else None
        if xP is not None:
            z, cm = ops.conv3x3_pre_bn_partials(xP, packed, x_slots)
        else:
            x_amax = aux.get("x_amax") if aux is not None else None
            z, cm = ops.conv3x3_fwd_bn_partials(x, packed, amax=x_amax) if training else (ops.conv3x3_auto(x, packed, 0, amax=x_amax), None)
        G = groups if (training and groups > 1) else 1
        Bz, C, Hz, Wz = z.shape
        Bg = Bz // G
        save_all = torch.empty((G, 4, C), dtype=torch.float32, device=z.device)
        want = bool(p16.get("want"))
        keep = bool(p16.get("keep_fp32")) or not want or ops.PRESPLIT_KEEP_FP32
        aP = None
        if want:
            aP = p16.get("out")
            if aP is None:
                aP = ops.p16_empty(Bz, C, Hz, Wz, z.device)
        head = p16.get("head_link")
        defer_head = bool(head is not None and training and G == 2 and not want and want_pool is None and z.dtype == torch.float32
                          and ops.HEAD_NORM and not ops.PRESPLIT_KEEP_FP32)
        a = torch.empty(z.shape, dtype=torch.float32, device=z.device) if (keep and not defer_head) else ops.fp32_placeholder(z.shape, z.device)
        parts2 = ops.p16_parts() == 2
        act_slots = ops.new_amax(z.device) if (want and parts2 and training) else None
        a_amax = ops.new_amax(z.device) if (not want and parts2) else None
        pooled = None
        if want_pool is not None and Hz % 2 == 0 and Wz % 2 == 0:
            if want_pool.get("p16"):
                pooled = (None, None, ops.p16_empty(Bz, C, Hz // 2, Wz // 2, z.device))
            else:
                pooled = (torch.empty((Bz, C, Hz // 2, Wz // 2), dtype=torch.float32, device=z.device), None, None)
        if training and cm is not None:
            ops.bn_train_coeffs(z[:Bg], gamma, beta, running_mean, running_var, momentum, eps, cm=(cm, 0, cm.shape[1] // G), save=save_all,
                                act_slots=act_slots, groups=G)
        else:
            for g in range(G):
                if training:
                    ops.bn_train_coeffs(z[g * Bg:(g + 1) * Bg], gamma, beta, running_mean, running_var, momentum, eps, save=save_all[g],
                                        act_slots=act_slots)
                else:
                    ops.bn_eval_coeffs(gamma, beta, running_mean, running_var, eps, save=save_all[g])
        gi = Bg if G > 1 else 0
        if defer_head:
            head["z"], head["save"] = z, save_all
            head["bwd_fuse"] = xP is not None
            a_amax = None
        elif pooled is not None:
            if not ops.bn_relu_apply_pool_split(z, save_all, aP, a if keep else None, pooled[2], pooled[0], slots=act_slots, group_images=gi):
                raise RuntimeError("onet_amd: pre-split BatchNorm + pooling pass refused a shape ops.pre_layer_ok accepted")
        elif aP is not None:
            ops.bn_relu_apply_split(z, save_all, aP, a=a if keep else None, slots=act_slots, group_images=gi)
        else:
            ops.bn_relu_apply(z, save_all, out=a, amax=a_amax, group_images=gi)
        p16["a"], p16["a_slots"], p16["a_amax"] = aP, act_slots, a_amax
        ctx.x_slots = x_slots
        ctx.up_link = p16.get("up_link")
        ctx.up_want = None if ctx.up_link is None else ctx.up_link.get("want")
        ctx.twin = ops.twin_src_of(x)
        ctx.head_link = head if defer_head else None
        below = (link_in.pop("z"), link_in.pop("save")) if (training and link_in is not None and "z" in link_in) else (None, None)
        ctx.save_for_backward(x, z, save_all, xP, *below)
        ctx.pre = True
        ctx.training = training
        ctx.packed = packed
        ctx.wshape = tuple(weight.shape)
        _record_versions(ctx, weight, gamma, beta)
        ctx.link_out = ctx.link_in = None
        if training and link_out is not None:
            link_out.clear()
            link_out.update(z=z, save=save_all)
            ctx.link_out = link_out
        if below[0] is not None:
            ctx.link_in = link_in
        if pooled is not None and link_out is not None:
            link_out["pooled"] = pooled
        return a

    @staticmethod
    def _retag_twin(ctx, x):
        tw = getattr(ctx, "twin", None)
        if tw is not None and x is not None and ops.twin_src_of(x) is None:
            x._onet_twin_src = [tw[0], tw[1], None]
        return x

    @staticmethod
    def _take_head_handoff(link, da):
        if link is None or "gl" not in link:
            return None
        rda, rec4, da_amax, gl = link.pop("da"), link.pop("rec4"), link.pop("da_amax", None), link.pop("gl")
        if not ops.is_placeholder(da) or rda.data_ptr() != da.data_ptr() or rda.shape != da.shape or rda.stride() != da.stride():
            raise RuntimeError("onet_amd: the head kept the gradient of the last activation unwritten, but autograd handed its unit "
                               "another tensor (a second consumer of that activation?)")
        return rec4, da_amax, gl

    @staticmethod
    def _backward_pre(ctx, da):
        x, z, save_all, xP, z_below, save_below = ctx.saved_tensors
        x = ConvBNReLUFn._retag_twin(ctx, x)
        need_x, need_w, need_g, need_b = ctx.needs_input_grad[:4]
        _check_versions(ctx, (True, True, False))
        pw, pg, pb = ctx.params
        aff = (ops.grad_slot_if_free(pg) if need_g else None, ops.grad_slot_if_free(pb) if need_b else None)
        rec4, da_amax = None, None
        lk = ctx.link_out
        if lk is not None and "rec4" in lk:
            rda, rec4, da_amax = lk.pop("da"), lk.pop("rec4", None), lk.pop("da_amax", None)
            lk.pop("rec", None)
            if rda.data_ptr() != da.data_ptr() or rda.shape != da.shape or rda.stride() != da.stride():
                rec4 = da_amax = None
        da_gl = None
        hand = ConvBNReLUFn._take_head_handoff(getattr(ctx, "head_link", None), da)
        if hand is not None:
            rec4, da_amax, da_gl = hand
        nones = (None,) * 12
        if xP is None:
            if need_w and not need_x and x.shape[1] <= 4 and ops.STEM_WGRAD_BN and (not ops.is_placeholder(x) or ops.twin_src_of(x) is not None):
                dw, dgamma, dbeta = ops.stem_wgrad_bn(x, da, z, save_all, ctx.training, ctx.wshape, affine_out=aff, rec4=rec4,
                                                      out=ops.grad_slot_if_free(pw))
                return (None, dw, (dgamma if need_g else None), (dbeta if need_b else None)) + nones
            dz, dgamma, dbeta = ops.bn_relu_bwd_groups(da, z, save_all, ctx.training, affine_out=aff, rec4=rec4)
            dw = ops.conv3x3_wgrad_auto(x, dz, ctx.wshape, out=ops.grad_slot_if_free(pw)) if need_w else None
            dx = ops.conv3x3_auto(dz, ctx.packed, 1) if need_x else None
            return (dx, dw, (dgamma if need_g else None), (dbeta if need_b else None)) + nones
        dzP, dz_slots, dgamma, dbeta = ops.bn_relu_bwd_split(da, z, save_all, ctx.training, need_affine_grads=(need_g or need_b),
                                                             affine_out=aff, rec4=rec4, da_amax=da_amax, da_gl=da_gl)
        s1, s2, sc = ops._slots3(getattr(ctx, "x_slots", None))
        dw = ops.conv3x3_split_wgrad_pre(xP, dzP, ctx.wshape, out=ops.grad_slot_if_free(pw), x_slots=s1, dz_slots=dz_slots, x_slots2=s2,
                                         split_ch=sc) if need_w else None
        dpack = ctx.packed.get_pack("split" if dzP.shape[3] == 2 else "plain16")[1]
        dx = None
        if need_x and z_below is not None and save_below is not None and ctx.training:
            fused = ops.conv3x3_split_dgrad_pre_bnreduce(dzP, dpack, ctx.wshape[1], z_below, save_below, slots=dz_slots,
                                                         always=dz_slots is not None, want_amax=ops.p16_parts() == 2)
            if fused is not None:
                dx, rec_below, am_below = fused
                ctx.link_in["da"], ctx.link_in["rec4"] = dx, rec_below
                if am_below is not None:
                    ctx.link_in["da_amax"] = am_below
        up = getattr(ctx, "up_link", None)
        if need_x and dx is None and up is not None and ctx.up_want and (dz_slots is not None or dzP.shape[3] == 1):
            C2, Ct = ctx.up_want
            bound = ops.conv3x3_dgrad_bound(pw, dz_slots, C2) if dzP.shape[3] == 2 else None
            dx, dyP = ops.conv3x3_split_dgrad_pre_slots(dzP, dpack, ctx.wshape[1], C2, bound, slots=dz_slots, always=dz_slots is not None)
            up["dyP"], up["dy_slots"], up["da"] = dyP, bound, dx
        if need_x and dx is None:
            dx = ops.conv3x3_split_pre(dzP, dpack, ctx.wshape[1], slots=dz_slots, always=dz_slots is not None)
        return (dx, dw, (dgamma if need_g else None), (dbeta if need_b else None)) + nones

    @staticmethod
    def backward(ctx, da):
        if ctx.pre:
            return ConvBNReLUFn._backward_pre(ctx, da)
        x, z, save_all, nz, nsave, z_below, save_below = ctx.saved_tensors
        x = ConvBNReLUFn._retag_twin(ctx, x)
        need_x, need_w, need_g, need_b = ctx.needs_input_grad[:4]
        _check_versions(ctx, (True, True, False))
        pw, pg, pb = ctx.params
        aff = (ops.grad_slot_if_free(pg) if need_g else None, ops.grad_slot_if_free(pb) if need_b else None)
        G = save_all.shape[0]
        rec = rec4 = None
        lk = ctx.link_out
        if lk is not None and ("rec" in lk or "rec4" in lk):
            rda, rec, rec4 = lk.pop("da"), lk.pop("rec", None), lk.pop("rec4", None)
            if rda.data_ptr() != da.data_ptr() or rda.shape != da.shape or rda.stride() != da.stride():
                rec = rec4 = None
        Bz, Cz, Hz, Wz = z.shape
        dz_amax = ops.new_amax(z.device) if (ops.grad_f16() and ops.conv_algo() in ("auto", "split", "bf16")
                                             and ops.split_enabled() and Wz >= 16) else None
        if G == 1:
            dz, dgamma, dbeta = ops.bn_relu_bwd(da, z, save_all[0], ctx.training, need_affine_grads=(need_g or need_b),
                                                affine_out=aff, red=None if rec is None else (rec, 0, rec.shape[1]),
                                                red4=None if rec4 is None else (rec4, 0, rec4.shape[0]), amax=dz_amax)
        else:
            Bg = z.shape[0] // G
            dz = torch.empty_like(z)
            dgamma = dbeta = None
            for g in range(G):
                sl = slice(g * Bg, (g + 1) * Bg)
                npg = 0 if rec is None else rec.shape[1] // G
                np4 = 0 if rec4 is None else rec4.shape[0] // G
                _, dgamma, dbeta = ops.bn_relu_bwd(da[sl], z[sl], save_all[g], ctx.training, need_affine_grads=True,
                                                   out=dz[sl], acc=None if g == 0 else (dgamma, dbeta),
                                                   affine_out=aff if g == 0 else None,
                                                   red=None if rec is None else (rec, g * npg, npg),
                                                   red4=None if rec4 is None else (rec4, g * np4, np4), amax=dz_amax)
        if need_w and nz is not None:
            dw = ops.conv3x3_split_wgrad(nz, dz, ctx.wshape, out=ops.grad_slot_if_free(pw), norm=nsave, dz_amax=dz_amax)
        else:
            dw = ops.conv3x3_wgrad_auto(x, dz, ctx.wshape, out=ops.grad_slot_if_free(pw), dz_amax=dz_amax) if need_w else None
        dx = None
        if need_x:
            lk = ctx.link_in
            fused = None
            if lk is not None and z_below is not None:
                fused = ops.conv3x3_dgrad_bnreduce(dz, ctx.packed, z_below, save_below)
            if fused is not None:
                dx, r = fused
                lk["da"], lk["rec"] = dx, r
            else:
                dx = ops.conv3x3_auto(dz, ctx.packed, 1, amax=dz_amax)
        return (dx, dw, (dgamma if need_g else None), (dbeta if need_b else None)) + (None,) * 12


@_carries_settings
class Conv3x3Fn(torch.autograd.Function):

    @staticmethod
    def forward(ctx, x, weight, packed):
        ops.require_gpu(x, weight)
        z = ops.conv3x3_auto(x, packed, 0)
        ctx.save_for_backward(x)
        ctx.packed = packed
        ctx.wshape = tuple(weight.shape)
        _record_versions(ctx, weight)
        return z

    @staticmethod
    def backward(ctx, dz):
        (x,) = ctx.saved_tensors
        _check_versions(ctx, (True,))
        dw = ops.conv3x3_wgrad_auto(x, dz, ctx.wshape) if ctx.needs_input_grad[1] else None
        dx = ops.conv3x3_auto(dz, ctx.packed, 1) if ctx.needs_input_grad[0] else None
        return dx, dw, None


@_carries_settings
class BNReLUFn(torch.autograd.Function):

    @staticmethod
    def forward(ctx, z, gamma, beta, running_mean, running_var, training, momentum, eps):
        ops.require_gpu(z, gamma, beta)
        if training:
            save = ops.bn_train_coeffs(z, gamma, beta, running_mean, running_var, momentum, eps)
        else:
            save = ops.bn_eval_coeffs(gamma, beta, running_mean, running_var, eps)
        a = ops.bn_relu_apply(z, save)
        ctx.save_for_backward(z, save)
        ctx.training = training
        return a

    @staticmethod
    def backward(ctx, da):
        z, save = ctx.saved_tensors
        dz, dgamma, dbeta = ops.bn_relu_bwd(da, z, save, ctx.training, True)
        return dz, dgamma, dbeta, None, None, None, None, None


@_carries_settings
class MaxPool2Fn(torch.autograd.Function):

    @staticmethod
    def forward(ctx, x):
        ops.require_gpu(x)
        y = ops.maxpool2_fwd(x)
        ctx.save_for_backward(x)
        return y

    @staticmethod
    def backward(ctx, dy):
        (x,) = ctx.saved_tensors
        return ops.maxpool2_bwd(x, dy)


@_carries_settings
class SkipPoolFn(torch.autograd.Function):

    @staticmethod
    def forward(ctx, x, returned=False, link=None, carry=None):
        ops.require_gpu(x)
        pooled = link.pop("pooled", None) if link is not None else None
        if pooled is not None and len(pooled) == 3:
            shp = (x.shape[0], x.shape[1], x.shape[2] // 2, x.shape[3] // 2)
            y = pooled[0] if pooled[0] is not None else ops.fp32_placeholder(shp, x.device)
            if carry is not None:
                carry["yP"] = pooled[2]
            ctx.pre = True
        elif pooled is not None and pooled[0] is not None and tuple(pooled[0].shape) == (x.shape[0], x.shape[1], x.shape[2] // 2, x.shape[3] // 2):
            y = pooled[0]
        else:
            y = ops.maxpool2_fwd(x)
        below = (link.pop("z"), link.pop("save")) if (link is not None and "z" in link) else (None, None)
        ctx.save_for_backward(x, *below)
        ctx.link = link if below[0] is not None else None
        return (x.view_as(x), y, x.view_as(x)) if returned else (x.view_as(x), y)

    @staticmethod
    def backward(ctx, g_skip, g_pool, g_ret=None):
        x, z, save = ctx.saved_tensors
        if g_pool is None:
            gs = [g for g in (g_skip, g_ret) if g is not None]
            return (sum(gs[1:], gs[0]) if gs else None), None, None, None
# ... 310 lines not shown
```

### onet_amd/ops.py

```python
from __future__ import annotations

import torch

from . import _lib

F32 = torch.float32


import os as _os
from collections import namedtuple as _namedtuple


def _flags_from_env():
    out = {}
    for item in _os.environ.get("ONET_FLAGS", "").split(","):
        if "=" in item:
            k, v = item.split("=", 1)
            out[k.strip()] = v.strip()
    return out


_FLAGS = _flags_from_env()


# ... 884 lines not shown
    zbs = out.stride(0) if B > 1 else Cout * H * W
    e0 = _prof_begin("conv_wino4_kernel")
    _lib.call("onet_conv3x3_winograd4_fwd", _p(x), xbs, _p(wq), _p(out), zbs, B, Cin, Cout, H, W, _stream())
    _prof_end("conv_wino4_kernel", 2.0 * B * H * W * Cin * Cout * 9, e0, 4.0 * (B * H * W * (Cin + Cout) + 9 * Cin * Cout))
    return out


def pack3x3_plain16(w):
    require_gpu(w)
    w = w.detach().contiguous()
    Cout, Cin = w.shape[0], w.shape[1]
    wf = torch.empty(Cin * 9 * Cout + 8, dtype=BF, device=w.device) if Cin % 16 == 0 else None
    wd = torch.empty((-(-Cout // 16) * 16) * 9 * Cin + 8, dtype=BF, device=w.device)
    _lib.call("onet_conv3x3_split_pack_weights", _p(w), _p(wf), _p(wd), None, Cout, Cin, 2, 2, _stream())
    return wf, wd


def pack3x3_split(w):
    require_gpu(w)
    w = w.detach().contiguous()
    Cout, Cin = w.shape[0], w.shape[1]
    f_fwd, f_dg = split_f16(), grad_f16() or presplit()
    wf = torch.empty(2 * Cin * 9 * Cout + 8, dtype=torch.float16 if f_fwd else BF, device=w.device) if Cin % 16 == 0 else None
    wd = torch.empty(2 * (-(-Cout // 16) * 16) * 9 * Cin + 8, dtype=torch.float16 if f_dg else BF, device=w.device)
    ws = torch.empty(AMAX_SLOTS, dtype=torch.int32, device=w.device) if (f_fwd or f_dg) else None
    _lib.call("onet_conv3x3_split_pack_weights", _p(w), _p(wf), _p(wd), _p(ws), Cout, Cin, int(f_fwd), int(f_dg), _stream())
    return wf, wd


class counting_batches:

    def __enter__(self):
        self.outer = getattr(_TLS, "counters", None)
        _TLS.counters = []
        return self

    def __exit__(self, *exc):
        pending, _TLS.counters = _TLS.counters, self.outer
        by_inc = {}
        for t, n in pending:
            by_inc.setdefault(n, []).append(t)
        for n, ts in by_inc.items():
            if len(ts) > 1 and all(t.is_cuda for t in ts):
                torch._foreach_add_(ts, n)
            else:
                for t in ts:
                    t.add_(n)
        return False


def count_batches(counter, n):
    pending = getattr(_TLS, "counters", None)
    if pending is None:
        counter.add_(n)
    else:
        pending.append((counter, n))


AMAX_SLOTS = 64 * 32


_AMAX_ARENA = {}
AMAX_ARENA_ROWS = 192


def amax_arena_reset(device):
    key = (device.type, device.index if device.index is not None else torch.cuda.current_device())
    ar = _AMAX_ARENA[key] = [torch.empty((AMAX_ARENA_ROWS, AMAX_SLOTS), dtype=torch.int32, device=device), 0]
    fill(ar[0].view(torch.float32), 0.0)


def new_amax(device):
    key = (device.type, device.index if device.index is not None else torch.cuda.current_device())
    ar = _AMAX_ARENA.get(key)
    if ar is not None and ar[1] < AMAX_ARENA_ROWS:
        ar[1] += 1
        return ar[0][ar[1] - 1]
    return torch.zeros(AMAX_SLOTS, dtype=torch.int32, device=device)


def absmax_slots(x):
    require_gpu(x)
    xc = x.contiguous()
    slots = new_amax(x.device)
    _lib.call("onet_absmax_slots", _p(xc), xc.numel(), _p(slots), _stream())
    return slots


def conv3x3_split(x, wq, Cout, out=None, norm=None, amax=None, always=False):
    if wq is None or not wq.is_cuda or wq.dtype not in (torch.bfloat16, torch.float16):
        raise TypeError("conv3x3_split: wq must be a split pack on the GPU (pack3x3_split)")
    f16 = int(wq.dtype == torch.float16)
    require_gpu(x)
    if norm is not None:
        require_gpu(norm)
        x, xbs = plane(x)
        B, Cin, H, W = x.shape
        if out is None:
            out = torch.empty((B, Cout, H, W), dtype=F32, device=x.device)
        e0 = _prof_begin("conv3x3_split_kernel")
        _lib.call("onet_conv3x3_split_fwd_norm", _p(x), xbs, _p(norm), norm.shape[0], _p(wq), f16, _p(amax) if f16 else None, _p(out),
                  out.stride(0) if B > 1 else Cout * H * W, None, B, Cin, Cout, H, W, _stream())
        _prof_end("conv3x3_split_kernel", 2.0 * B * H * W * Cin * Cout * 9, e0, 4.0 * (B * H * W * (Cin + Cout) + 9 * Cin * Cout))
        return out
    x, xbs = plane(x)
    if x.data_ptr() % 16 or xbs % 4:
        x = x.contiguous()
        xbs = x.stride(0) if x.shape[0] > 1 else x[0].numel()
    B, Cin, H, W = x.shape
    if out is None:
        out = torch.empty((B, Cout, H, W), dtype=F32, device=x.device)
    zbs = out.stride(0) if B > 1 else Cout * H * W
    if f16 and always and amax is None:
        amax = absmax_slots(x)
    e0 = _prof_begin("conv3x3_split_kernel")
    if f16:
        _lib.call("onet_conv3x3_split_conv_amax", _p(x), xbs, _p(amax), int(always), _p(wq), _p(out), zbs, None, B, Cin, Cout, H, W, _stream())
    else:
        _lib.call("onet_conv3x3_split_fwd", _p(x), xbs, _p(wq), 0, _p(out), zbs, B, Cin, Cout, H, W, _stream())
    _prof_end("conv3x3_split_kernel", 2.0 * B * H * W * Cin * Cout * 9, e0, 4.0 * (B * H * W * (Cin + Cout) + 9 * Cin * Cout))
    return out


def split_pack_act(x, f16=True, scale=1.0, out=None, parts=2, slots=None):
    require_gpu(x)
    x, xbs = plane(x)
    B, C, H, W = x.shape
    if out is not None:
        parts = out.shape[3]
    if out is None:
        out = torch.empty((B, C // 8, H, parts, W, 8), dtype=torch.float16 if (f16 and parts == 2) else BF, device=x.device)
    _lib.call("onet_split_pack_act", _p(x), xbs, _p(out), _pbs(out), B, C, H, W, 2 if parts == 1 else int(f16), float(scale), _p(slots),
              _stream())
    return out


def conv3x3_split_pre(xs, wq, Cout, out=None, slots=None, always=False, stats=None, slots2=None, split_ch=0, z16=False):
    if wq is None or not wq.is_cuda or wq.dtype not in (torch.bfloat16, torch.float16) or xs.dtype != wq.dtype:
        raise TypeError("conv3x3_split_pre: xs and wq must be split packs of the same 16-bit type on the GPU")
    B, C8, H, two, W, eight = xs.shape
    f16 = 2 if two == 1 else int(wq.dtype == torch.float16)
    Cin = C8 * 8
    if out is None:
        out = torch.empty((B, Cout, H, W), dtype=BF if (z16 and two == 1) else F32, device=xs.device)
    e0 = _prof_begin("conv3x3_split_pre_kernel")
    _lib.call("onet_conv3x3_split_fwd_pre", _p(xs), _pbs(xs), _p(slots), int(always), _p(slots2), int(split_ch if slots2 is not None or slots is not None else 0),
              _p(wq), f16, _p(out), _z16(out),
              out.stride(0) if B > 1 else Cout * H * W, _p(stats), B, Cin, Cout, H, W, _stream())
    _prof_end("conv3x3_split_pre_kernel", 2.0 * B * H * W * Cin * Cout * 9, e0,
              B * H * W * (2.0 * two * Cin + out.element_size() * Cout) + 2.0 * two * 9 * Cin * Cout)
    return out


def conv3x3_split_dgrad_pre_bnreduce(dzP, wq, Cout, z_prev, save_prev, slots=None, always=False, want_amax=False):
    if not FUSE_BN_REDUCE or sync_bn() or not FUSE_DGRAD_REDUCE:
        return None
    B, C8, H, two, W, _ = dzP.shape
    Cin = C8 * 8
    G = save_prev.shape[0]
    if tuple(z_prev.shape) != (B, Cout, H, W) or B % G or not save_prev.is_contiguous() or wq.dtype != dzP.dtype:
        return None
    lib = _lib.load()
    nparts = int(lib.onet_conv3x3_split_pre_nparts(B, H, W))
    z_prev, zbs = plane(z_prev)
    if nparts <= 0 or nparts % G or (zbs & 3) or (z_prev.data_ptr() & 15):
        return None
    f16 = 2 if two == 1 else int(wq.dtype == torch.float16)
    da = torch.empty((B, Cout, H, W), dtype=F32, device=dzP.device)
    rec4 = torch.empty((nparts, Cout, 4), dtype=F32, device=dzP.device)
    am = new_amax(dzP.device) if want_amax else None
    e0 = _prof_begin("conv3x3_split_pre_kernel")
    rc = lib.onet_conv3x3_split_dgrad_pre_bnreduce(_p(dzP), _pbs(dzP), _p(slots), int(always), _p(wq), f16, _p(da), Cout * H * W, _p(z_prev), _z16(z_prev), zbs,
                                                   _p(save_prev), B // G if G > 1 else 0, _p(rec4), _p(am), B, Cin, Cout, H, W, _stream())
    _prof_end("conv3x3_split_pre_kernel", 2.0 * B * H * W * Cin * Cout * 9 if rc == 0 else 0.0, e0,
              (B * H * W * (2.0 * two * Cin + (4.0 + z_prev.element_size()) * Cout) + 2.0 * two * 9 * Cin * Cout) if rc == 0 else 0.0)
    if rc < 0:
        raise _lib.OnetHipError(f"onet_conv3x3_split_dgrad_pre_bnreduce failed ({rc}): {_lib.last_error()}")
    return (da, rec4, am) if rc == 0 else None


def eval_layer_ok(B, Cin, Cout, H, W):
    return _eval_domain("fp16x2", "full", B, Cin, Cout, H, W)


def _eval_domain(fmt, mode, B, Cin, Cout, H, W):
    fp16 = fmt == "fp16x2"
    if not presplit() or (fp16 and p16_parts() != 2) or Cin % (16 if fp16 else 32) or Cout % 64:
        return False
    if mode == "full":
        map_ok = full_tiles(H, W) and H * W < 2 ** 24
    elif mode == "ragged":
        map_ok = W > 16 and _ragged_map(H, W) and (W >= RAGGED_MIN_W or full_tiles(H, W))
    elif mode == "anymap":
        map_ok = H > 0 and W > 16 and W >= max(RAGGED_MIN_W, ANYMAP_MIN_W) and H * W < 2 ** 24 and not _ragged_map(H, W)
    else:
        map_ok = B > 0 and H > 0 and W >= max(PAIRS_MIN_W, 1)
    if not map_ok:
        return False
    if fp16 and mode != "pairs":
        return conv3x3_algo(B, Cin, Cout, H, W) == "split"
    if not _in_buffer_range(Cin, Cout, H, W):
        return False
    if conv_algo() in (("split",) if fp16 else ("bf16", "split")):
        return True
    tiles = -(-B // 2) * -(-H // 16) if mode == "pairs" else B * -(-H // 16) * -(-W // 32)
    return tiles * (Cout // 64) >= (n_cu() * 3) // 4


def eval_layer_ok_bf16(B, Cin, Cout, H, W):
    return _eval_domain("bf16", "full", B, Cin, Cout, H, W)


def full_tiles(H, W):
    return W >= 32 and W % 32 == 0 and H % 16 == 0


def _ragged_map(H, W):
    return H > 0 and W > 0 and H % 2 == 0 and W % 4 == 0 and H * W < 2 ** 24


RAGGED_MIN_W = int(_FLAGS.get("RAGGED_MIN_W", 20))


def eval_layer_ok_ragged(B, Cin, Cout, H, W):
    return _eval_domain("bf16", "ragged", B, Cin, Cout, H, W)


ANYMAP_MIN_W = int(_FLAGS.get("ANYMAP_MIN_W", RAGGED_MIN_W))


def eval_layer_ok_anymap(B, Cin, Cout, H, W):
    return eval_layer_ok_ragged(B, Cin, Cout, H, W) or _eval_domain("bf16", "anymap", B, Cin, Cout, H, W)


PAIRS_MIN_W = int(_FLAGS.get("PAIRS_MIN_W", 9))
PAIRS_SINGLE = _flag("PAIRS_SINGLE", False)


def eval_layer_ok_pairs(B, Cin, Cout, H, W):
    if W > 16:
        return eval_layer_ok_anymap(B, Cin, Cout, H, W)
    return _eval_domain("bf16", "pairs", B, Cin, Cout, H, W)


def eval_layer_ok_ragged_fp16(B, Cin, Cout, H, W):
    if full_tiles(H, W):
        return eval_layer_ok(B, Cin, Cout, H, W)
    return _eval_domain("fp16x2", "ragged", B, Cin, Cout, H, W)


def eval_layer_ok_pairs_fp16(B, Cin, Cout, H, W):
    if W > 16:
        return eval_layer_ok_ragged_fp16(B, Cin, Cout, H, W)
    return _eval_domain("fp16x2", "pairs", B, Cin, Cout, H, W)


def conv3x3_act_bound(weight, save, x_amax, x_amax2=None, split_ch=0):
    w = weight.detach()
    w = w if w.is_contiguous() else w.contiguous()
    slots = new_amax(w.device)
    _lib.call("onet_conv3x3_act_bound", _p(w), w.shape[0], w.shape[1], _p(save), _p(x_amax), _p(x_amax2), int(split_ch if x_amax2 is not None else 0),
              _p(slots), _stream())
    return slots


EVAL_ENTRIES = {
    ("fp16x2", "full", "act"): ("onet_conv3x3_split_fwd_pre_act", "conv3x3_split_pre_act_kernel"),
    ("fp16x2", "full", "act_pool"): ("onet_conv3x3_split_fwd_pre_act_pool", "conv3x3_split_pre_act_pool_kernel"),
    ("fp16x2", "full", "head"): ("onet_conv3x3_split_fwd_pre_head", "conv3x3_split_pre_head_kernel"),
    ("fp16x2", "ragged", "act"): ("onet_conv3x3_split_fwd_pre_act_ragged", "conv3x3_split_pre_act_kernel"),
    ("fp16x2", "ragged", "act_pool"): ("onet_conv3x3_split_fwd_pre_act_pool_ragged", "conv3x3_split_pre_act_pool_kernel"),
    ("fp16x2", "ragged", "head"): ("onet_conv3x3_split_fwd_pre_head_ragged", "conv3x3_split_pre_head_kernel"),
    ("fp16x2", "ragged", "plain"): ("onet_conv3x3_split_fwd_pre_plain_ragged", "conv3x3_split_pre_kernel"),
    ("fp16x2", "pairs", "act"): ("onet_conv3x3_split_fwd_pre_act_pairs", "conv3x3_split_pre_act_pairs_kernel"),
    ("bf16", "full", "act"): ("onet_conv3x3_plain16_fwd_pre_act", "conv3x3_pre16_act_kernel"),
    ("bf16", "full", "act_pool"): ("onet_conv3x3_plain16_fwd_pre_act_pool", "conv3x3_pre16_act_pool_kernel"),
    ("bf16", "full", "head"): ("onet_conv3x3_plain16_fwd_pre_head", "conv3x3_pre16_head_kernel"),
    ("bf16", "ragged", "act"): ("onet_conv3x3_plain16_fwd_pre_act_ragged", "conv3x3_pre16_act_kernel"),
    ("bf16", "ragged", "act_pool"): ("onet_conv3x3_plain16_fwd_pre_act_pool_ragged", "conv3x3_pre16_act_pool_kernel"),
    ("bf16", "ragged", "head"): ("onet_conv3x3_plain16_fwd_pre_head_ragged", "conv3x3_pre16_head_kernel"),
    ("bf16", "ragged", "plain"): ("onet_conv3x3_plain16_fwd_pre_plain_ragged", "conv3x3_split_pre_kernel"),
    ("bf16", "anymap", "act"): ("onet_conv3x3_plain16_fwd_pre_act_anymap", "conv3x3_pre16_act_kernel"),
    ("bf16", "anymap", "act_pool"): ("onet_conv3x3_plain16_fwd_pre_act_pool_anymap", "conv3x3_pre16_act_pool_kernel"),
    ("bf16", "pairs", "act"): ("onet_conv3x3_plain16_fwd_pre_act_pairs", "conv3x3_pre16_act_pairs_kernel"),
}


_EVAL_NAMES = {key: entry[len("onet_"):].replace("_fwd_pre_", "_pre_") for key, (entry, _) in EVAL_ENTRIES.items()}


def eval_conv_name(fmt, mode, epilogue):
    return _EVAL_NAMES.get((fmt, mode, epilogue))


def eval_conv(fmt, mode, epilogue, xs, wq, Cout, save=None, L=None, aP_slots=None, out=None, slots=None, slots2=None, split_ch=0,
              a_amax=None, a=None, yP=None, y=None):
    entry, kind = EVAL_ENTRIES[fmt, mode, epilogue]
    two = fmt == "fp16x2"
    dt = torch.float16 if two else BF
    if wq is None or not wq.is_cuda or wq.dtype != dt or xs.dtype != dt or xs.shape[3] != 1 + two:
        raise TypeError(f"{eval_conv_name(fmt, mode, epilogue)}: xs and wq must be " + ("fp16 (hi | mid) split" if two else "one-part bf16") + " packs on the GPU")
    if PAIRS_SINGLE and (fmt, mode) == ("bf16", "pairs"):
        mode = "anymap"
        entry, kind = EVAL_ENTRIES[fmt, mode, epilogue]
    x_slots = (_p(slots), 0, _p(slots2), int(split_ch if slots2 is not None or slots is not None else 0)) if two else ()
    if epilogue == "head":
        return _pre_head(entry, kind, 1 + two, xs, wq, Cout, save, L, out, x_slots)
    if epilogue == "plain":
        return _pre_plain(entry, kind, 1 + two, xs, wq, Cout, out, x_slots)
    return _pre_act(entry, kind, 1 + two, mode, xs, wq, Cout, save, out, a_amax, a, x_slots, (_p(aP_slots),) if two else (),
                    pooled=(yP, y) if epilogue == "act_pool" else None)


def _pre_act(entry, kind, two, mode, xs, wq, Cout, save, out, a_amax, a, extra_in, extra_out, pooled=None):
    B, C8, H, _, W, _ = xs.shape
    Cin = C8 * 8
    if pooled is not None and pooled[0] is None and pooled[1] is None:
        raise ValueError(f"{entry[len('onet_'):]}: a pooled destination is required (yP, y or both)")
    if mode in ("anymap", "pairs"):
        map_ok = 0 < H * W < 2 ** 24 and (mode == "anymap" or W <= 16)
    else:
        map_ok = _ragged_map(H, W) if mode == "ragged" else full_tiles(H, W)
    if not map_ok or Cin % (16 if two == 2 else 32) or Cout % 64:
        return None
    if out is None:
        out = p16_empty(B, Cout, H, W, xs.device, parts=two)
    n = Cout * H * W
    pool_args, pool_bytes = (), 0.0
    if pooled is not None:
        yP, y = pooled
        pool_args = (_p(yP), 0 if yP is None else _pbs(yP), _p(y), 0 if y is None else (y.stride(0) if B > 1 else Cout * (H // 2) * (W // 2)))
# ... 1014 lines not shown
```

Baseline: 601.3.

## Fuse stem weight-gradient tap sums into the next layer's dgrad+BN-reduce kernel

Adds a STEM variant of the fused fp16 dgrad/BN-reduce kernel. It loads the single-channel input patch (with the twin complement transform) into LDS and accumulates the 3x3 tap products of dy and the normalized activation per block, writing per-tile tap records. A small finish kernel then combines these with the BN coefficients to form the stem's weight gradient. This skips materializing the stem's activation gradient and running a separate stem wgrad/BN backward pass, at the cost of extra register pressure, LDS traffic and arithmetic in the fused kernel.

```diff
diff --git a/include/onet_hip_stem.h b/include/onet_hip_stem.h
--- /dev/null
+++ b/include/onet_hip_stem.h
@@ -0,0 +1,20 @@
+#ifndef ONET_HIP_STEM_H
+#define ONET_HIP_STEM_H
+#include <stdint.h>
+#ifdef __cplusplus
+extern "C" {
+#endif
+
+int onet_conv3x3_split_dgrad_pre_stem(const void* dzs, int64_t dzs_bs, const void* dz_amax, int scale_always, const void* wq, int wq_f16,
+                                      const float* z_prev, int64_t z_bs, const float* save, int group_images, float* rec4, const float* x,
+                                      int64_t x_bs, int twin_B, float twin_bias, float* tap_rec, int B, int Cin, int Cout, int H, int W,
+                                      void* stream);
+int64_t onet_conv3x3_stem_taps_ws_bytes(int B, int H);
+int onet_conv3x3_stem_taps_finish(const float* tap_rec, const float* x, int64_t x_bs, int twin_B, float twin_bias, const float* save,
+                                  const float* coef, int group_images, float* dw, void* ws, int64_t ws_bytes, int B, int Cout, int H, int W,
+                                  void* stream);
+
+#ifdef __cplusplus
+}
+#endif
+#endif
diff --git a/onet_amd/_lib.py b/onet_amd/_lib.py
--- a/onet_amd/_lib.py
+++ b/onet_amd/_lib.py
@@ -14,6 +14,7 @@
 UPMAP_HEADER = os.path.join(os.path.dirname(HERE), "include", "onet_hip_upmap.h")
 SPLIT_PAIRS_HEADER = os.path.join(os.path.dirname(HERE), "include", "onet_hip_split_pairs.h")
 OPTIM_HEADER = os.path.join(os.path.dirname(HERE), "include", "onet_hip_optim.h")
+STEM_HEADER = os.path.join(os.path.dirname(HERE), "include", "onet_hip_stem.h")
 LIBPATH = os.environ.get("ONET_HIP_LIB") or os.path.join(HERE, "libonet_hip.so")
 
 _CT = {
@@ -70,7 +71,7 @@
         _build.build()
     lib = ctypes.CDLL(LIBPATH)
     _protos = {}
-    for header in (HEADER, EVAL_HEADER, RAGGED_HEADER, RAGGED_SPLIT_HEADER, ANYMAP_HEADER, PAIRS_HEADER, UPMAP_HEADER, SPLIT_PAIRS_HEADER, OPTIM_HEADER):
+    for header in (HEADER, EVAL_HEADER, RAGGED_HEADER, RAGGED_SPLIT_HEADER, ANYMAP_HEADER, PAIRS_HEADER, UPMAP_HEADER, SPLIT_PAIRS_HEADER, OPTIM_HEADER, STEM_HEADER):
         protos = parse_header(header)
         for name, (restype, argtypes, _) in protos.items():
             try:
diff --git a/onet_amd/build.py b/onet_amd/build.py
--- a/onet_amd/build.py
+++ b/onet_amd/build.py
@@ -14,7 +14,7 @@
         return True
     t = os.path.getmtime(LIB)
     deps = [os.path.join(CSRC, f) for f in os.listdir(CSRC) if f.endswith((".hip", ".cpp", ".hpp"))] + \
-        [os.path.join(HERE, "..", "include", h) for h in ("onet_hip.h", "onet_hip_eval.h", "onet_hip_ragged.h", "onet_hip_ragged_split.h", "onet_hip_anymap.h", "onet_hip_pairs.h", "onet_hip_upmap.h", "onet_hip_split_pairs.h", "onet_hip_optim.h")]
+        [os.path.join(HERE, "..", "include", h) for h in ("onet_hip.h", "onet_hip_eval.h", "onet_hip_ragged.h", "onet_hip_ragged_split.h", "onet_hip_anymap.h", "onet_hip_pairs.h", "onet_hip_upmap.h", "onet_hip_split_pairs.h", "onet_hip_optim.h", "onet_hip_stem.h")]
     return any(os.path.getmtime(d) > t for d in deps)
 
 
diff --git a/onet_amd/csrc/conv_split.hip b/onet_amd/csrc/conv_split.hip
--- a/onet_amd/csrc/conv_split.hip
+++ b/onet_amd/csrc/conv_split.hip
@@ -559,12 +559,12 @@
     int z16 = 0, rd_z16 = 0;
     void* zP = nullptr;
     int64_t zP_bs = 0;
-    int zP_ch0 = 0;
-    const unsigned* zP_slots = nullptr;
-    const float* act_save = nullptr;
+    union { int zP_ch0 = 0; int sm_twin_B; };
+    union { const unsigned* zP_slots = nullptr; float sm_twin_bias; };
+    union { const float* act_save = nullptr; const float* sm_x; };
     unsigned* act_amax = nullptr;
-    float* act_a = nullptr;
-    int64_t act_a_bs = 0;
+    union { float* act_a = nullptr; float* sm_rec; };
+    union { int64_t act_a_bs = 0; int64_t sm_x_bs; };
     union { const float* hd_L = nullptr; void* pl_P; };
     union { int64_t hd_L_bs = 0; int64_t pl_P_bs; };
     union { float* hd_V = nullptr; float* pl_y; };
@@ -1026,9 +1026,11 @@
     const unsigned r0 = (unsigned)__shfl_xor((int)(o4 ? Alo : Blo), 4, 64), r1 = (unsigned)__shfl_xor((int)(o4 ? Ahi : Bhi), 4, 64);
     return o4 ? u32x4s{r0, r1, Blo, Bhi} : u32x4s{Alo, Ahi, r0, r1};
 }
-template <bool ST, int PM, bool W16, bool RD = false, bool ACT = false, bool HEAD = false, bool POOL = false, bool RAG = false, bool ANY = false>
+template <bool ST, int PM, bool W16, bool RD = false, bool ACT = false, bool HEAD = false, bool POOL = false, bool RAG = false, bool ANY = false,
+          bool STEM = false>
 __global__ __launch_bounds__(512, 2) void conv3x3_pre16_kernel(SpPreArgs a) {
     constexpr bool F16 = PM == 1;
+    static_assert(!STEM || (RD && PM == 1 && !W16), "conv3x3_pre16_kernel: the stem tap sums ride on the fused reduce of an fp16 (hi | mid) input gradient");
     static_assert(!ANY || (ACT && PM == 2 && !RAG), "conv3x3_pre16_kernel: the any-map instance is the one-part activation epilogue's");
     static_assert(!POOL || ACT, "conv3x3_pre16_kernel: the pooled stores ride on the activation epilogue");
     static_assert(!RAG || (POOL && PM == 2), "conv3x3_pre16_kernel: the ragged instance is the one-part pooled epilogue's");
@@ -1043,6 +1045,7 @@
     constexpr int CH_OFF = W16 ? 18 : 16;
     constexpr int NSTEP = PM == 2 ? 9 : 14;
     constexpr bool PAIRS = W16 && ACT;
+    [[maybe_unused]] constexpr int SM_PS = 36;
     extern __shared__ __attribute__((aligned(16))) unsigned char smem_s[];
     u32x4s* lds = reinterpret_cast<u32x4s*>(smem_s);
 
@@ -1365,6 +1368,24 @@
         }
         f32x4s zr[4][NT][2];
         const float* rd_sv = nullptr;
+        [[maybe_unused]] float xp0 = 0.f, xp1 = 0.f, pivot = 0.f;
+        [[maybe_unused]] int ti = tid;
+        if constexpr (STEM) {
+            asm volatile("" : "+v"(ti));
+            const bool comp = a.sm_twin_B > 0 && b >= a.sm_twin_B;
+            const float* xb = a.sm_x + (int64_t)(comp ? b - a.sm_twin_B : b) * a.sm_x_bs;
+            const int py = y0 - 1, pxl = x0 - 1;
+            auto px = [&](int i) __attribute__((always_inline)) {
+                const int yy = py + i / IN_COLS, xx = pxl + i % IN_COLS;
+                const bool ok = i < C::NPIX && yy >= 0 && yy < a.H && xx >= 0 && xx < a.W;
+                float v = ok ? xb[(int64_t)yy * a.W + xx] : 0.f;
+                if (comp && ok) v = fminf(fmaxf(1.f - v + a.sm_twin_bias, 0.f), 1.f);
+                return v;
+            };
+            pivot = px((C::ROWS / 2) * IN_COLS + 16);
+            xp0 = px(ti) - pivot;
+            xp1 = px(ti + 512) - pivot;
+        }
         if constexpr (RD) {
             const int img0 = W16 ? 2 * b : b;
             rd_sv = a.rd_save + (int64_t)(a.rd_gimg ? img0 / a.rd_gimg : 0) * 4 * a.Cout;
@@ -1389,8 +1410,17 @@
                         zr[ct][n][ch] = zz;
                     }
             __builtin_amdgcn_sched_barrier(0);
-        }
-        {
+            if constexpr (STEM) {
+                float* xpatch = reinterpret_cast<float*>(lds + (buf ^ 1) * BUF) + 8 * 64 * 21;
+                xpatch[ti / IN_COLS * SM_PS + ti % IN_COLS] = xp0;
+                if (ti < C::NPIX - 512) xpatch[(ti + 512) / IN_COLS * SM_PS + (ti + 512) % IN_COLS] = xp1;
+                if (ti == 0) xpatch[C::IN_ROWS * SM_PS] = pivot;
+                asm volatile("s_waitcnt lgkmcnt(0)" ::: "memory");
+                __builtin_amdgcn_s_barrier();
+                __builtin_amdgcn_sched_barrier(0);
+            }
+        }
+        if constexpr (!STEM) {
             const int half = r16 >> 3, c8 = r16 & 7;
             float* zb = a.z + (int64_t)(W16 ? 2 * b + half : b) * a.z_bs;
             const int xo = (W16 ? 0 : x0 + 16 * half) + 4 * lq;
@@ -1520,12 +1550,15 @@
         if constexpr (RD) {
             __builtin_amdgcn_sched_barrier(0);
             float* sc = reinterpret_cast<float*>(lds + (buf ^ 1) * BUF);
+            constexpr int SCW = STEM ? 21 : 2;
+            [[maybe_unused]] float* const xpatch = sc + 8 * 64 * SCW;
             float vmax = 0.f;
 #pragma unroll
             for (int ct = 0; ct < 4; ++ct) {
                 const int co = co0 + ct * 16 + r16, cc = min(co, a.Cout - 1);
                 const float mean = rd_sv[cc], invstd = rd_sv[a.Cout + cc], scl = rd_sv[2 * a.Cout + cc], sh = rd_sv[3 * a.Cout + cc];
                 float s1 = 0.f, s2 = 0.f;
+                [[maybe_unused]] float sd = 0.f;
 #pragma unroll
                 for (int n = 0; n < NT; ++n)
 #pragma unroll
@@ -1539,7 +1572,14 @@
                                 s1 += dy;
                                 s2 = fmaf(dy, d * invstd, s2);
                                 vmax = fmaxf(vmax, fabsf(da));
+                                if constexpr (STEM) {
+                                    sd += d;
+                                    acc[ct][n][ch][r] = dy;
+                                    zr[ct][n][ch][r] = d;
+                                }
                             }
+                        } else if constexpr (STEM) {
+                            acc[ct][n][ch] = zr[ct][n][ch] = f32x4s{0.f, 0.f, 0.f, 0.f};
                         }
                     }
                 s1 += __shfl_xor(s1, 16, 64);
@@ -1547,11 +1587,59 @@
                 s1 += __shfl_xor(s1, 32, 64);
                 s2 += __shfl_xor(s2, 32, 64);
                 if (lq == 0) {
-                    sc[(wn * 64 + ct * 16 + r16) * 2] = s1;
-                    sc[(wn * 64 + ct * 16 + r16) * 2 + 1] = s2;
-                }
-            }
-            if (a.rd_amax) {
+                    sc[(wn * 64 + ct * 16 + r16) * SCW] = s1;
+                    sc[(wn * 64 + ct * 16 + r16) * SCW + 1] = s2;
+                }
+                if constexpr (STEM) {
+                    sd += __shfl_xor(sd, 16, 64);
+                    sd += __shfl_xor(sd, 32, 64);
+                    if (lq == 0) sc[(wn * 64 + ct * 16 + r16) * SCW + 2] = sd;
+                }
+            }
+            if constexpr (STEM) {
+                auto red4 = [&](float v0, float v1, float v2, float v3) __attribute__((always_inline)) {
+                    asm("s_nop 1\n\tv_permlane32_swap_b32 %0, %1" : "+v"(v0), "+v"(v2));
+                    asm("s_nop 1\n\tv_permlane32_swap_b32 %0, %1" : "+v"(v1), "+v"(v3));
+                    float r1 = v0 + v2, r2 = v1 + v3;
+                    asm("s_nop 1\n\tv_permlane16_swap_b32 %0, %1" : "+v"(r1), "+v"(r2));
+                    return r1 + r2;
+                };
+                float* const mine = sc + (wn * 64 + lane) * SCW;
+#pragma unroll
+                for (int ky = 0; ky < 3; ++ky) {
+                    float xw[NT][2][6];
+#pragma unroll
+                    for (int n = 0; n < NT; ++n)
+#pragma unroll
+                        for (int ch = 0; ch < 2; ++ch) {
+                            const float* p = xpatch + (wn * NT + n + ky) * SM_PS + 16 * ch + 4 * lq;
+                            const f32x4s v = *reinterpret_cast<const f32x4s*>(p);
+                            const float2 w = *reinterpret_cast<const float2*>(p + 4);
+                            xw[n][ch][0] = v[0]; xw[n][ch][1] = v[1]; xw[n][ch][2] = v[2]; xw[n][ch][3] = v[3];
+                            xw[n][ch][4] = w.x; xw[n][ch][5] = w.y;
+                        }
+#pragma unroll
+                    for (int kx = 0; kx < 3; ++kx) {
+                        float ta[4], tb[4];
+#pragma unroll
+                        for (int ct = 0; ct < 4; ++ct) {
+                            ta[ct] = tb[ct] = 0.f;
+#pragma unroll
+                            for (int n = 0; n < NT; ++n)
+#pragma unroll
+                                for (int ch = 0; ch < 2; ++ch)
+#pragma unroll
+                                    for (int r = 0; r < 4; ++r) {
+                                        ta[ct] = fmaf(acc[ct][n][ch][r], xw[n][ch][r + kx], ta[ct]);
+                                        tb[ct] = fmaf(zr[ct][n][ch][r], xw[n][ch][r + kx], tb[ct]);
+                                    }
+                        }
+                        mine[3 + 3 * ky + kx] = red4(ta[0], ta[1], ta[2], ta[3]);
+                        mine[12 + 3 * ky + kx] = red4(tb[0], tb[1], tb[2], tb[3]);
+                    }
+                }
+            }
+            if (!STEM && a.rd_amax) {
 #pragma unroll
                 for (int o = 32; o > 0; o >>= 1) vmax = fmaxf(vmax, __shfl_xor(vmax, o, 64));
                 if (lane == 0 && vmax == vmax) atomicMax(a.rd_amax + ((blockIdx.x * 8 + wn) & (AMAX_SLOTS - 1)) * AMAX_STRIDE, __builtin_bit_cast(unsigned, vmax));
@@ -1561,8 +1649,8 @@
                 double t1 = 0.0, t2 = 0.0;
 #pragma unroll
                 for (int w = 0; w < 8; ++w) {
-                    t1 += (double)sc[(w * 64 + tid) * 2];
-                    t2 += (double)sc[(w * 64 + tid) * 2 + 1];
+                    t1 += (double)sc[(w * 64 + tid) * SCW];
+                    t2 += (double)sc[(w * 64 + tid) * SCW + 1];
                 }
                 const int64_t blk = ((int64_t)b * a.tilesY + ty) * a.tilesX + tx;
                 float* o = a.rd_rec + (blk * a.Cout + co0 + tid) * 4;
@@ -1571,6 +1659,25 @@
                 o[2] = (float)t2;
                 o[3] = (float)(t2 - (double)o[2]);
             }
+            if constexpr (STEM) {
+                int co = tid & 63;
+                asm volatile("" : "+v"(co));
+                if (co0 + co < a.Cout) {
+                    const int64_t blk = ((int64_t)b * a.tilesY + ty) * a.tilesX + tx;
+                    for (int k = wn; k < 18; k += 8) {
+                        const int jb = k < 9 ? 0 : 2;
+                        double base = 0.0, t = 0.0;
+#pragma unroll
+                        for (int w = 0; w < 8; ++w) {
+                            base += (double)sc[(w * 64 + co) * SCW + jb];
+                            t += (double)sc[(w * 64 + co) * SCW + 3 + k];
+                        }
+                        const double s = t + (double)xpatch[C::IN_ROWS * SM_PS] * base;
+                        const float hi = (float)s;
+                        reinterpret_cast<float2*>(a.sm_rec)[(blk * 18 + k) * a.Cout + co0 + co] = make_float2(hi, (float)(s - (double)hi));
+                    }
+                }
+            }
             __syncthreads();
         }
     }
@@ -1587,7 +1694,8 @@
     return check_launch(name);
 }
 
-template <bool ST, int PM, bool W16, bool RD = false, bool ACT = false, bool HEAD = false, bool POOL = false, bool RAG = false, bool ANY = false>
+template <bool ST, int PM, bool W16, bool RD = false, bool ACT = false, bool HEAD = false, bool POOL = false, bool RAG = false, bool ANY = false,
+          bool STEM = false>
 int launch_split_pre(SpPreArgs a, hipStream_t st) {
     using C = SpPreCfg<W16>;
     const int LDS_BYTES = C::LDS_BYTES + (ST ? C::NW * 64 * 2 * 4 : 0) + (ACT || HEAD ? 2 * 3 * 64 * 4 : 0);
@@ -1605,7 +1713,7 @@
     constexpr bool P16 = RD || PM == 2 || (ST && !W16) || HEAD;
     void (*kern)(SpPreArgs);
     static_assert(!ANY || P16, "launch_split_pre: the any-map instance exists on the 16x16x32 kernel alone");
-    if constexpr (P16) kern = conv3x3_pre16_kernel<ST, PM, W16, RD, ACT, HEAD, POOL, RAG, ANY>;
+    if constexpr (P16) kern = conv3x3_pre16_kernel<ST, PM, W16, RD, ACT, HEAD, POOL, RAG, ANY, STEM>;
     else kern = conv3x3_split_pre_kernel<ST, PM, W16, ACT, POOL, RAG>;
     static PerDeviceOnce attr_once;
     return sp_launch_persistent(kern, attr_once, LDS_BYTES, tiles, C::NW * 64,
@@ -2419,6 +2527,33 @@
     return wq_f16 ? launch_split_pre<false, 1, false, true>(a, st) : launch_split_pre<false, 0, false, true>(a, st);
 }
 
+int onet_conv3x3_split_dgrad_pre_stem(const void* dzs, int64_t dzs_bs, const void* dz_amax, int scale_always, const void* wq, int wq_f16,
+                                      const float* z_prev, int64_t z_bs, const float* save, int group_images, float* rec4, const float* x,
+                                      int64_t x_bs, int twin_B, float twin_bias, float* tap_rec, int B, int Cin, int Cout, int H, int W,
+                                      void* stream) {
+    ONET_REQUIRE(dzs && wq && z_prev && save && rec4 && x && tap_rec, "conv3x3_split_dgrad_pre_stem: null pointer");
+    if (wq_f16 != 1 || Cout != 64 || W == 16 || (W % 32) || onet_conv3x3_split_pre_nparts(B, H, W) <= 0 || Cin / 16 < 4) return 1;
+    ONET_REQUIRE(B > 0 && Cin > 0, "conv3x3_split_dgrad_pre_stem: bad shape");
+    ONET_REQUIRE(group_images >= 0 && (group_images == 0 || B % group_images == 0), "conv3x3_split_dgrad_pre_stem: bad statistics groups");
+    ONET_REQUIRE(twin_B == 0 || 2 * twin_B == B, "conv3x3_split_dgrad_pre_stem: a twin batch holds twin_B = B / 2 images in memory");
+    if (const int rc = pre_operand_checks("conv3x3_split_dgrad_pre_stem", dzs, dzs_bs, wq_f16, Cin, Cout, H, W)) return rc;
+    ONET_REQUIRE((z_bs & 3) == 0 && (reinterpret_cast<uintptr_t>(z_prev) & 15) == 0, "conv3x3_split_dgrad_pre_stem: 16-byte aligned rows required");
+    ONET_REQUIRE(z_bs >= (int64_t)Cout * H * W && x_bs >= (int64_t)H * W, "conv3x3_split_dgrad_pre_stem: batch stride too small");
+    ONET_REQUIRE((reinterpret_cast<uintptr_t>(tap_rec) & 7) == 0, "conv3x3_split_dgrad_pre_stem: 8-byte aligned tap records required");
+    SpPreArgs a{dzs, dzs_bs, (const __bf16*)wq, nullptr, 0, B, Cin, Cout, H, W, 0, 0, 0, nullptr, (const unsigned*)dz_amax, scale_always, nullptr, 0};
+    a.rd_z = z_prev;
+    a.rd_z_bs = z_bs;
+    a.rd_save = save;
+    a.rd_gimg = group_images;
+    a.rd_rec = rec4;
+    a.sm_x = x;
+    a.sm_x_bs = x_bs;
+    a.sm_twin_B = twin_B;
+    a.sm_twin_bias = twin_bias;
+    a.sm_rec = tap_rec;
+    return launch_split_pre<false, 1, false, true, false, false, false, false, false, true>(a, as_stream(stream));
+}
+
 int onet_conv3x3_split_dgrad_pre_slots(const void* dzs, int64_t dzs_bs, const void* dz_amax, int scale_always, const void* wq, int wq_f16,
                                        float* da, int64_t da_bs, void* daP, int64_t daP_bs, int ch0, const void* daP_amax, int B, int Cin,
                                        int Cout, int H, int W, void* stream) {
diff --git a/onet_amd/csrc/stem.hip b/onet_amd/csrc/stem.hip
--- a/onet_amd/csrc/stem.hip
+++ b/onet_amd/csrc/stem.hip
@@ -128,9 +128,126 @@
     return n < (1 << 30) ? (int)n : 0;
 }
 
+constexpr int TAP_N = 18 * 64, TAP_PW = TAP_N + 16;
+
+struct StemTapArgs {
+    const float* rec;
+    const float* x;
+    int64_t x_bs;
+    double* part;
+    int B, H, W, tilesX, tilesY, P, twin_B;
+    float twin_bias;
+};
+
+__global__ __launch_bounds__(384) void stem_taps_gather_kernel(StemTapArgs a) {
+    __shared__ double red[6][9];
+    const int b = blockIdx.x / a.P, p = blockIdx.x % a.P;
+    const int ty0 = p * a.tilesY / a.P, ty1 = (p + 1) * a.tilesY / a.P;
+    const int tid = threadIdx.x, lane = tid & 63, wid = tid >> 6;
+    const float2* r = reinterpret_cast<const float2*>(a.rec) + ((int64_t)b * a.tilesY + ty0) * a.tilesX * TAP_N;
+    const int ntl = (ty1 - ty0) * a.tilesX;
+    double acc[3] = {0.0, 0.0, 0.0};
+#pragma unroll 4
+    for (int i = 0; i < ntl; ++i)
+#pragma unroll
+        for (int e = 0; e < 3; ++e) {
+            const float2 v = r[(int64_t)i * TAP_N + tid + 384 * e];
+            acc[e] += (double)v.x + (double)v.y;
+        }
+    double* out = a.part + (int64_t)blockIdx.x * TAP_PW;
+#pragma unroll
+    for (int e = 0; e < 3; ++e) out[tid + 384 * e] = acc[e];
+
+    const bool comp = a.twin_B > 0 && b >= a.twin_B;
+    const float* xb = a.x + (int64_t)(comp ? b - a.twin_B : b) * a.x_bs;
+    const int ya = ty0 * 16, npx = (ty1 - ty0) * 16 * a.W;
+    double sx[9];
+#pragma unroll
+    for (int t = 0; t < 9; ++t) sx[t] = 0.0;
+    for (int i = tid; i < npx; i += 384) {
+        const int y = ya + i / a.W, x = i % a.W;
+        float v = xb[(int64_t)y * a.W + x];
+        if (comp) v = fminf(fmaxf(1.f - v + a.twin_bias, 0.f), 1.f);
+#pragma unroll
+        for (int t = 0; t < 9; ++t) {
+            const int yo = y - t / 3 + 1, xo = x - t % 3 + 1;
+            if (yo >= 0 && yo < a.H && xo >= 0 && xo < a.W) sx[t] += (double)v;
+        }
+    }
+#pragma unroll
+    for (int t = 0; t < 9; ++t) {
+        double s = sx[t];
+#pragma unroll
+        for (int o = 32; o > 0; o >>= 1) s += __shfl_xor(s, o, 64);
+        if (lane == 0) red[wid][t] = s;
+    }
+    __syncthreads();
+    if (tid < 9) out[TAP_N + tid] = ((red[0][tid] + red[1][tid]) + (red[2][tid] + red[3][tid])) + (red[4][tid] + red[5][tid]);
+}
+
+__global__ __launch_bounds__(1024) void stem_taps_finish_kernel(const double* __restrict__ part, int nper, int G, const float* __restrict__ save,
+                                                                const float* __restrict__ coef, float* __restrict__ dw) {
+    __shared__ double sh[3][16][64];
+    const int t = blockIdx.x, co = threadIdx.x & 63, sl = threadIdx.x >> 6;
+    double total = 0.0;
+    for (int g = 0; g < G; ++g) {
+        double s_dy = 0.0, s_d = 0.0, s_x = 0.0;
+        for (int q = sl; q < nper; q += 16) {
+            const double* pp = part + ((int64_t)g * nper + q) * TAP_PW;
+            s_dy += pp[t * 64 + co];
+            s_d += pp[(9 + t) * 64 + co];
+            s_x += pp[TAP_N + t];
+        }
+        sh[0][sl][co] = s_dy;
+        sh[1][sl][co] = s_d;
+        sh[2][sl][co] = s_x;
+        __syncthreads();
+        if (sl == 0) {
+            s_dy = s_d = s_x = 0.0;
+            for (int k = 0; k < 16; ++k) {
+                s_dy += sh[0][k][co];
+                s_d += sh[1][k][co];
+                s_x += sh[2][k][co];
+            }
+            const float* sv = save + (int64_t)g * 4 * 64;
+            const float* cf = coef + (int64_t)g * 4 * 64;
+            const double c1 = (double)cf[co] + (double)cf[64 + co], c2 = (double)cf[128 + co] + (double)cf[192 + co];
+            total += (double)sv[128 + co] * (s_dy - c1 * s_x - c2 * (double)sv[64 + co] * s_d);
+        }
+        __syncthreads();
+    }
+    if (sl == 0) dw[co * 9 + t] = (float)total;
+}
+
+int stem_taps_parts(int B, int H) { return std::max(1, std::min(H / 16, 256 / std::max(B, 1))); }
+
 }
 
 extern "C" {
+
+int64_t onet_conv3x3_stem_taps_ws_bytes(int B, int H) { return (int64_t)B * stem_taps_parts(B, H) * TAP_PW * 8; }
+
+int onet_conv3x3_stem_taps_finish(const float* tap_rec, const float* x, int64_t x_bs, int twin_B, float twin_bias, const float* save,
+                                  const float* coef, int group_images, float* dw, void* ws, int64_t ws_bytes, int B, int Cout, int H, int W,
+                                  void* stream) {
+    ONET_REQUIRE(tap_rec && x && save && coef && dw && ws, "conv3x3_stem_taps_finish: null pointer");
+    ONET_REQUIRE(B > 0 && Cout == 64 && H > 0 && W > 0 && (H % 16) == 0 && (W % 32) == 0,
+                 "conv3x3_stem_taps_finish: needs Cout == 64 and a map made of full 16 x 32 tiles");
+    ONET_REQUIRE(group_images >= 0 && (group_images == 0 || B % group_images == 0), "conv3x3_stem_taps_finish: bad statistics groups");
+    ONET_REQUIRE(twin_B == 0 || 2 * twin_B == B, "conv3x3_stem_taps_finish: a twin batch holds twin_B = B / 2 images in memory");
+    ONET_REQUIRE(x_bs >= (int64_t)H * W, "conv3x3_stem_taps_finish: batch stride too small");
+    ONET_REQUIRE((reinterpret_cast<uintptr_t>(tap_rec) & 7) == 0 && (reinterpret_cast<uintptr_t>(ws) & 7) == 0,
+                 "conv3x3_stem_taps_finish: 8-byte aligned records and workspace required");
+    const int P = stem_taps_parts(B, H);
+    ONET_REQUIRE(ws_bytes >= onet_conv3x3_stem_taps_ws_bytes(B, H), "conv3x3_stem_taps_finish: workspace %lld < %lld bytes", (long long)ws_bytes,
+                 (long long)onet_conv3x3_stem_taps_ws_bytes(B, H));
+    const int G = group_images ? B / group_images : 1;
+    StemTapArgs a{tap_rec, x, x_bs, (double*)ws, B, H, W, W / 32, H / 16, P, twin_B, twin_bias};
+    hipLaunchKernelGGL(stem_taps_gather_kernel, dim3((unsigned)(B * P)), dim3(384), 0, as_stream(stream), a);
+    if (const int rc = check_launch("stem_taps_gather_kernel")) return rc;
+    hipLaunchKernelGGL(stem_taps_finish_kernel, dim3(9), dim3(1024), 0, as_stream(stream), (const double*)ws, (B / G) * P, G, save, coef, dw);
+    return check_launch("stem_taps_finish_kernel");
+}
 
 int onet_conv3x3_stem_nparts(int B, int Cin, int Cout, int H, int W) { return stem_nparts(B, Cin, Cout, H, W); }
 
diff --git a/onet_amd/functional.py b/onet_amd/functional.py
--- a/onet_amd/functional.py
+++ b/onet_amd/functional.py
@@ -191,6 +191,8 @@
         ctx.twin = ops.twin_src_of(x)
         ctx.head_link = head if defer_head else None
         below = (link_in.pop("z"), link_in.pop("save")) if (training and link_in is not None and "z" in link_in) else (None, None)
+        stem = link_in.pop("stem_x", None) if link_in is not None else None
+        ctx.stem_below = stem if (below[0] is not None and xP is not None) else None
         ctx.save_for_backward(x, z, save_all, xP, *below)
         ctx.pre = True
         ctx.training = training
@@ -201,6 +203,8 @@
         if training and link_out is not None:
             link_out.clear()
             link_out.update(z=z, save=save_all)
+            if xP is None and z.dtype == torch.float32 and not ctx.needs_input_grad[0] and ops.stem_bwd_fuse_ok(x):
+                link_out["stem_x"] = (x, ops.twin_src_of(x))
             ctx.link_out = link_out
         if below[0] is not None:
             ctx.link_in = link_in
@@ -224,6 +228,16 @@
             raise RuntimeError("onet_amd: the head kept the gradient of the last activation unwritten, but autograd handed its unit "
                                "another tensor (a second consumer of that activation?)")
         return rec4, da_amax, gl
+
+    @staticmethod
+    def _take_stem_handoff(link, da):
+        if link is None or "stem_taps" not in link:
+            return None
+        rda, rec4, taps = link.pop("da"), link.pop("rec4"), link.pop("stem_taps")
+        if not ops.is_placeholder(da) or rda.data_ptr() != da.data_ptr() or rda.shape != da.shape or rda.stride() != da.stride():
+            raise RuntimeError("onet_amd: the gradient of the stem's activation was kept unwritten, but autograd handed the stem "
+                               "another tensor (a second consumer of that activation?)")
+        return rec4, taps
 
     @staticmethod
     def _backward_pre(ctx, da):
@@ -235,6 +249,13 @@
         aff = (ops.grad_slot_if_free(pg) if need_g else None, ops.grad_slot_if_free(pb) if need_b else None)
         rec4, da_amax = None, None
         lk = ctx.link_out
+        stem_hand = ConvBNReLUFn._take_stem_handoff(lk, da)
+        if stem_hand is not None:
+            if xP is not None or need_x or not need_w or not ctx.training:
+                raise RuntimeError("onet_amd: tap records were handed to a unit that is not a training-mode stem without an input gradient")
+            dw, dgamma, dbeta = ops.stem_taps_finish(stem_hand[1], x, z, save_all, True, ctx.wshape, affine_out=aff, rec4=stem_hand[0],
+                                                     out=ops.grad_slot_if_free(pw))
+            return (None, dw, (dgamma if need_g else None), (dbeta if need_b else None)) + (None,) * 12
         if lk is not None and "rec4" in lk:
             rda, rec4, da_amax = lk.pop("da"), lk.pop("rec4", None), lk.pop("da_amax", None)
             lk.pop("rec", None)
@@ -261,14 +282,18 @@
                                          split_ch=sc) if need_w else None
         dpack = ctx.packed.get_pack("split" if dzP.shape[3] == 2 else "plain16")[1]
         dx = None
+        stem = getattr(ctx, "stem_below", None)
         if need_x and z_below is not None and save_below is not None and ctx.training:
+            kw = {} if stem is None else {"stem": stem}
             fused = ops.conv3x3_split_dgrad_pre_bnreduce(dzP, dpack, ctx.wshape[1], z_below, save_below, slots=dz_slots,
-                                                         always=dz_slots is not None, want_amax=ops.p16_parts() == 2)
+                                                         always=dz_slots is not None, want_amax=ops.p16_parts() == 2, **kw)
             if fused is not None:
-                dx, rec_below, am_below = fused
+                dx, rec_below, am_below = fused[:3]
                 ctx.link_in["da"], ctx.link_in["rec4"] = dx, rec_below
                 if am_below is not None:
                     ctx.link_in["da_amax"] = am_below
+                if len(fused) > 3 and fused[3] is not None:
+                    ctx.link_in["stem_taps"] = fused[3]
         up = getattr(ctx, "up_link", None)
         if need_x and dx is None and up is not None and ctx.up_want and (dz_slots is not None or dzP.shape[3] == 1):
             C2, Ct = ctx.up_want
diff --git a/onet_amd/ops.py b/onet_amd/ops.py
--- a/onet_amd/ops.py
+++ b/onet_amd/ops.py
@@ -1060,9 +1060,14 @@
     return out
 
 
-def conv3x3_split_dgrad_pre_bnreduce(dzP, wq, Cout, z_prev, save_prev, slots=None, always=False, want_amax=False):
+def conv3x3_split_dgrad_pre_bnreduce(dzP, wq, Cout, z_prev, save_prev, slots=None, always=False, want_amax=False, stem=None):
     if not FUSE_BN_REDUCE or sync_bn() or not FUSE_DGRAD_REDUCE:
         return None
+    if stem is not None:
+        got = conv3x3_split_dgrad_pre_stem(dzP, wq, Cout, z_prev, save_prev, stem[0], twin=stem[1], slots=slots, always=always) \
+            if stem_bwd_fuse_ok(stem[0]) else None
+        if got is not None:
+            return got[0], got[1], None, got[2]
     B, C8, H, two, W, _ = dzP.shape
     Cin = C8 * 8
     G = save_prev.shape[0]
@@ -1084,7 +1089,67 @@
               (B * H * W * (2.0 * two * Cin + (4.0 + z_prev.element_size()) * Cout) + 2.0 * two * 9 * Cin * Cout) if rc == 0 else 0.0)
     if rc < 0:
         raise _lib.OnetHipError(f"onet_conv3x3_split_dgrad_pre_bnreduce failed ({rc}): {_lib.last_error()}")
-    return (da, rec4, am) if rc == 0 else None
+    if rc != 0:
+        return None
+    return (da, rec4, am) if stem is None else (da, rec4, am, None)
+
+
+STEM_BWD_FUSE = _flag("STEM_BWD_FUSE", True)
+
+
+def stem_bwd_fuse_ok(x):
+    if not (STEM_BWD_FUSE and STEM_WGRAD_BN and FUSE_BN_REDUCE and FUSE_DGRAD_REDUCE) or sync_bn() or not presplit() or p16_parts() != 2:
+        return False
+    if x.dim() != 4 or x.shape[1] != 1 or x.requires_grad or x.dtype != F32 or not x.is_cuda:
+        return False
+    return (not is_placeholder(x)) or twin_src_of(x) is not None
+
+
+def conv3x3_split_dgrad_pre_stem(dzP, wq, Cout, z_prev, save_prev, x, twin=None, slots=None, always=False):
+    B, C8, H, two, W, _ = dzP.shape
+    Cin = C8 * 8
+    G = save_prev.shape[0]
+    if two != 2 or wq.dtype != torch.float16 or dzP.dtype != wq.dtype or Cout != 64 or z_prev.dtype != F32:
+        return None
+    if tuple(z_prev.shape) != (B, Cout, H, W) or B % G or not save_prev.is_contiguous():
+        return None
+    xs = twin[0] if twin is not None else x
+    if xs.dtype != F32 or tuple(xs.shape) != ((B // 2 if twin is not None else B), 1, H, W) or (twin is not None and B % 2):
+        return None
+    lib = _lib.load()
+    nparts = int(lib.onet_conv3x3_split_pre_nparts(B, H, W))
+    z_prev, zbs = plane(z_prev)
+    if nparts <= 0 or nparts % G or (zbs & 3) or (z_prev.data_ptr() & 15):
+        return None
+    xs, xbs = plane(xs)
+    rec4 = torch.empty((nparts, Cout, 4), dtype=F32, device=dzP.device)
+    taps = torch.empty((nparts, 18, Cout, 2), dtype=F32, device=dzP.device)
+    e0 = _prof_begin("conv3x3_split_pre_kernel")
+    rc = lib.onet_conv3x3_split_dgrad_pre_stem(_p(dzP), _pbs(dzP), _p(slots), int(always), _p(wq), 1, _p(z_prev), zbs, _p(save_prev),
+                                               B // G if G > 1 else 0, _p(rec4), _p(xs), xbs, B // 2 if twin is not None else 0,
+                                               float(twin[1]) if twin is not None else 0.0, _p(taps), B, Cin, Cout, H, W, _stream())
+    _prof_end("conv3x3_split_pre_kernel", 2.0 * B * H * W * Cin * Cout * 9 if rc == 0 else 0.0, e0,
+              (B * H * W * (2.0 * two * Cin + 4.0 * Cout + 4.0) + 2.0 * two * 9 * Cin * Cout + 4.0 * taps.numel()) if rc == 0 else 0.0)
+    if rc < 0:
+        raise _lib.OnetHipError(f"onet_conv3x3_split_dgrad_pre_stem failed ({rc}): {_lib.last_error()}")
+    return (fp32_placeholder((B, Cout, H, W), dzP.device), rec4, taps) if rc == 0 else None
+
+
+def stem_taps_finish(taps, x, z, save_all, training, dw_shape, affine_out=None, rec4=None, out=None, twin=None):
+    if twin is None:
+        twin = twin_src_of(x)
+    B, Cout, H, W = z.shape
+    xs, xbs = plane(twin[0] if twin is not None else x)
+    G = save_all.shape[0]
+    assert training and rec4 is not None and taps.is_contiguous() and tuple(taps.shape[1:]) == (18, 64, 2) and Cout == 64
+    coef, dgamma, dbeta = _bn_bwd_groups(None, 0, z, 0, save_all, True, affine_out, rec4, None, None)
+    dw = torch.empty(dw_shape, dtype=F32, device=z.device) if out is None else out
+    assert dw.is_contiguous() and dw.numel() == 9 * Cout
+    ws = workspace(_lib.load().onet_conv3x3_stem_taps_ws_bytes(B, H), z.device)
+    _lib.call("onet_conv3x3_stem_taps_finish", _p(taps), _p(xs), xbs, B // 2 if twin is not None else 0,
+              float(twin[1]) if twin is not None else 0.0, _p(save_all), _p(coef), B // G if G > 1 else 0, _p(dw), _p(ws), ws.numel() * 4,
+              B, Cout, H, W, _stream(), nbytes=4.0 * (taps.numel() + xs.numel()))
+    return dw, dgamma, dbeta
 
 
 def eval_layer_ok(B, Cin, Cout, H, W):
```

New measurement: 605.8, median of 6. Within noise of the previous version (+0.7%).
